# MichaelWoodhams/IQ-TREE

Hardware: AMD Instinct MI355X
Metric: million pattern-node partial-likelihood updates/sec (higher is better)
Workload: dtype f64; 1 GPU; DNA 50 taxa x 100000 patterns/GPU, GTR+G4, fixed tree: clearAllPartialLH + full traversal + root-branch lnL; ntaxa=50, patterns_per_gpu=100000, patterns_total=100000, nstates=4, ncat=4, parallelism=patterns sharded over 1 GPU(s), 1 RCCL all-reduce/step

## Files before the change

### include/iqhip.h

```cpp
#ifndef IQHIP_H_
#define IQHIP_H_

#include <stddef.h>
#include <stdint.h>

#ifdef __cplusplus
extern "C" {
#endif

#define IQHIP_ABI_VERSION 2

enum {
    IQHIP_OK = 0,
    IQHIP_ERR_NO_DEVICE = 1,
    IQHIP_ERR_INVALID = 2,
    IQHIP_ERR_UNSUPPORTED = 3,
    IQHIP_ERR_HIP = 4,
    IQHIP_ERR_NOMEM = 5
};

typedef struct iqhip_engine iqhip_engine;

typedef struct iqhip_node_op {
    uint64_t dst_key;
// ... 190 lines not shown
int iqhip_debug_pair_timing(iqhip_engine *e, double *counts_ms, double *solve_ms);

typedef struct iqhip_quartet_result {
    double  logl[3];
    double  len[3][5];
    int32_t nsweeps[3], neval[3], status[3], _pad;
} iqhip_quartet_result;
int iqhip_quartet_cells(iqhip_engine *e, const int32_t *quartets , int nq,
                        double *cells , int32_t *nother );
int iqhip_quartet_likelihoods(iqhip_engine *e, const int32_t *quartets, int nq,
                              const double *const_invar ,
                              double x1, double x2, double xacc, int max_steps, double diverge_frac,
                              int iterations, double tolerance, iqhip_quartet_result *results);
int iqhip_debug_quartet_timing(iqhip_engine *e, double *cells_ms, double *solve_ms);

typedef struct iqhip_bionj_step { int32_t a, b; double la, lb, lambda; } iqhip_bionj_step;
int iqhip_bionj(iqhip_engine *e, int n, const double *dist , const double *var ,
                iqhip_bionj_step *steps , int32_t *last , double *last_len );
int iqhip_debug_bionj_timing(iqhip_engine *e, double *ms, int64_t *launches);

typedef struct iqhip_pars_op { int32_t dst, left, right, _pad; } iqhip_pars_op;
int iqhip_pars_init(iqhip_engine *e, const uint8_t *informative , int nvectors, int64_t *nsites);
int iqhip_pars_update(iqhip_engine *e, const iqhip_pars_op *ops, int nops);
int iqhip_pars_branch_scores(iqhip_engine *e, const int32_t *ends , int nbranch, int32_t *score,
                             int32_t *subst );
int iqhip_pars_insert_scores(iqhip_engine *e, const int32_t *ends, int nbranch, int32_t taxon,
                             int32_t *score , int32_t *best, int32_t *best_score);
int iqhip_pars_shape(iqhip_engine *e, int64_t *nsites, int64_t *nwords, int *nvectors);
int iqhip_pars_fetch(iqhip_engine *e, int32_t slot, uint32_t *out );
int iqhip_debug_pars_levels(int ntaxa, int nvectors, const uint8_t *valid , const iqhip_pars_op *ops,
                            int nops, int32_t *level);
int iqhip_debug_pars_timing(iqhip_engine *e, double *ms , int64_t *counts , int reset);
int iqhip_pars_insert_scores_batch(iqhip_engine *e, const int32_t *ends ,
                                   const int32_t *seg_start , int nseg,
                                   const int32_t *taxon , int32_t *score ,
                                   int32_t *best , int32_t *best_score );
int iqhip_debug_pars_batch_timing(iqhip_engine *e, double *ms , int64_t *counts ,
                                  int reset);

enum { IQHIP_PARS_SPR_NO_SCORE = 1 };
#define IQHIP_PARS_SPR_MAX_RADIUS 10
typedef struct iqhip_pars_spr_step { int32_t parent, side, target, flags; } iqhip_pars_spr_step;
typedef struct iqhip_pars_spr_job { int32_t subtree, first_step, nsteps, _pad; } iqhip_pars_spr_job;
int iqhip_pars_spr_scan(iqhip_engine *e, const iqhip_pars_spr_job *jobs, int njobs, const iqhip_pars_spr_step *steps,
                        int nsteps, int32_t *score , int32_t *best_step ,
                        int32_t *best_score , int32_t *best_job);
int iqhip_debug_pars_spr_check(int ntaxa, int nvectors, const uint8_t *valid ,
                               const iqhip_pars_spr_job *jobs, int njobs, const iqhip_pars_spr_step *steps, int nsteps,
                               int32_t *depth );
int iqhip_debug_pars_spr_timing(iqhip_engine *e, double *ms , int64_t *counts , int reset);

int iqhip_upload_partial(iqhip_engine *e, uint64_t key, const double *partial_lh,
                         const int16_t *scale_num);

int iqhip_timing_enable(iqhip_engine *e, int on);
int iqhip_timing_read(iqhip_engine *e, double *avg_ms, int64_t *launches, int reset);
int iqhip_timing_plan_bytes(iqhip_engine *e, double *stored, double *loaded);
int iqhip_timing_collective_read(iqhip_engine *e, double *avg_us, int64_t *count, int reset);

int iqhip_debug_cherry_tables(iqhip_engine *e, int64_t *tables_built, int64_t *ops_from_tables);

#define IQHIP_PATH_NEWTON_ONE_LAUNCH 0
#define IQHIP_PATH_NEWTON_CHAIN 1
#define IQHIP_PATH_SWEEP_PERSISTENT 2
#define IQHIP_PATH_SWEEP_PER_STEP 3
#define IQHIP_PATH_SWEEP_SEQUENTIAL 4
#define IQHIP_PATH_NEWTON_FALLBACK 5
#define IQHIP_PATH_NSLOTS 6
int iqhip_debug_path_counts(iqhip_engine *e, int64_t *out, int n);

int iqhip_debug_create_planner(iqhip_engine **out, int nstates , int ncat, int64_t nptn, int ntaxa,
                               int num_cus, int state_unknown, int nclass);
int iqhip_debug_plan(iqhip_engine *e, const iqhip_node_op *ops, int nops);
#define IQHIP_PLAN_SHAPE_NSLOTS 28
int iqhip_debug_plan_shape(iqhip_engine *e, int64_t *out, int n);
#define IQHIP_PLAN_LAYOUT_NSLOTS 8
int iqhip_debug_plan_layout(iqhip_engine *e, int32_t *out, int nops);

int iqhip_debug_pair_children(iqhip_engine *e, int64_t *ops_removed, int64_t *slabs_expanded, int64_t *last_plan_removed);
int iqhip_debug_pair_rows(iqhip_engine *e, int64_t *slots_in_use, int64_t *restarts, int64_t *kept_real_for_lack_of_a_row);
int iqhip_debug_planner_plain_taxa(iqhip_engine *e, const uint8_t *plain);
int iqhip_debug_plan_removed(iqhip_engine *e, int32_t *out, int nrows);

void iqhip_debug_memory(int64_t *device_bytes, int64_t *host_bytes);
void iqhip_debug_fail_alloc(int nth);

typedef struct iqhip_partition iqhip_partition;
int iqhip_partition_create(iqhip_partition **out, iqhip_engine *const *members, int nparts);
void iqhip_partition_destroy(iqhip_partition *g);
int iqhip_partition_set_rates(iqhip_partition *g, const double *rate );
int iqhip_partition_newton_branch(iqhip_partition *g, double xguess, double x1, double x2, double xacc, int max_steps,
                                  double *optx, double *d2l, int *nsteps, double *part_lnl );
int iqhip_partition_lnl_from_theta(iqhip_partition *g, double x, double *part_lnl );
int iqhip_partition_traverse_lnl(iqhip_partition *g, const iqhip_node_op *ops, int nops, iqhip_branch_end a,
                                 iqhip_branch_end b, double len, const double *scale ,
                                 double *part_lnl );
int iqhip_partition_optimize_branch_batch(iqhip_partition *g, const iqhip_branch_task *tasks, int ntasks,
                                          iqhip_branch_result *results,
                                          double *part_lnl );
int iqhip_debug_partition_timing(iqhip_partition *g, double *ms ,
                                 int64_t *launches);

int iqhip_partition_ptnlh_reserve(iqhip_partition *g, int nrows);
int iqhip_partition_optimize_branch_batch_rows(iqhip_partition *g, const iqhip_branch_task *tasks, int ntasks,
                                               iqhip_branch_result *results,
                                               double *part_lnl ,
                                               const int32_t *rows );
int iqhip_partition_ptnlh_rell(iqhip_partition *g, const int32_t *rows, int nrows, int nsamples,
                               double *out );
int iqhip_partition_ufboot_init(iqhip_partition *g, int nsamples);
int iqhip_partition_ufboot_update(iqhip_partition *g, const iqhip_ufboot_tree *trees, int ntrees, double epsilon,
                                  double logl_cutoff, int64_t *counts , double *min_orig_logl );
int iqhip_partition_ufboot_fetch(iqhip_partition *g, double *boot_logl, double *boot_orig_logl, int32_t *boot_counts,
                                 int64_t *boot_tree);
int iqhip_debug_partition_ufboot_timing(iqhip_partition *g, double *ms , int64_t *launches);

int iqhip_partition_pair_distances(iqhip_partition *g, const double *init, double x1, double x2, double xacc, int max_steps,
                                   double *dist, double *d2l, int32_t *nsteps);
int iqhip_debug_partition_pair_timing(iqhip_partition *g, double *counts_ms, double *solve_ms);

#ifdef __cplusplus
}
#endif
#endif
```

### iq-tree_amd/__init__.py

```python
import ctypes as C
import os

import numpy as np

_HERE = os.path.dirname(os.path.abspath(__file__))
LIB_DIR = os.environ.get("IQHIP_LIB_DIR") or os.path.join(_HERE, "lib")
REPO_ROOT = os.path.dirname(_HERE)

IQHIP_SYMBOLS = [
    "iqhip_last_error", "iqhip_abi_version", "iqhip_device_count", "iqhip_create", "iqhip_destroy",
    "iqhip_set_stream", "iqhip_reserve", "iqhip_release", "iqhip_rekey", "iqhip_set_alignment",
    "iqhip_set_ptn_freq", "iqhip_set_ptn_invar", "iqhip_set_ascertainment", "iqhip_set_model", "iqhip_update_partials",
    "iqhip_branch_lnl", "iqhip_traverse_lnl", "iqhip_compute_theta", "iqhip_derv",
    "iqhip_lnl_from_theta", "iqhip_newton_branch", "iqhip_optimize_branch", "iqhip_bind_result_buffer", "iqhip_result_device_ptr",
    "iqhip_result_capacity", "iqhip_traverse_lnl_async", "iqhip_derv_async", "iqhip_result_read",
    "iqhip_synchronize", "iqhip_fetch_scale_num", "iqhip_fetch_pattern_lh", "iqhip_fetch_partial",
    "iqhip_fetch_theta", "iqhip_upload_partial", "iqhip_timing_enable", "iqhip_timing_read",
    "iqhip_fetch_pattern_lh_scaled", "iqhip_set_boot_samples", "iqhip_rell", "iqhip_rell_async",
    "iqhip_set_mixture_model", "iqhip_pattern_lh_cat", "iqhip_optimize_branch_batch",
    "iqhip_em_posteriors", "iqhip_em_fetch_posteriors", "iqhip_em_site_rates", "iqhip_em_objective", "iqhip_debug_em_timing",
    "iqhip_mix_class_lh", "iqhip_mix_weights_em", "iqhip_mix_posteriors", "iqhip_debug_mix_timing",
    "iqhip_class_lnl", "iqhip_debug_class_lnl_timing",
    "iqhip_create_sharded", "iqhip_num_shards", "iqhip_shard_range", "iqhip_comm_unique_id", "iqhip_comm_init_rank",
    "iqhip_comm_size", "iqhip_update_partials_async", "iqhip_lnl_from_theta_async",
    "iqhip_newton_host_init", "iqhip_newton_host_update", "iqhip_newton_host_result",
    "iqhip_debug_create_planner", "iqhip_debug_plan", "iqhip_timing_plan_bytes", "iqhip_timing_collective_read", "iqhip_optimize_sweep", "iqhip_debug_cherry_tables",
    "iqhip_debug_path_counts", "iqhip_debug_plan_shape", "iqhip_debug_plan_layout", "iqhip_debug_pair_children", "iqhip_debug_pair_rows", "iqhip_debug_planner_plain_taxa", "iqhip_debug_plan_removed", "iqhip_debug_memory", "iqhip_debug_fail_alloc",
    "iqhip_ptnlh_reserve", "iqhip_ptnlh_put_current", "iqhip_ptnlh_fetch", "iqhip_optimize_branch_batch_rows",
    "iqhip_branch_tests", "iqhip_ptnlh_rell",
    "iqhip_ptnlh_upload", "iqhip_gen_boot_samples", "iqhip_ptnlh_diff_variance", "iqhip_tree_tests", "iqhip_multiscale_bp",
    "iqhip_pair_counts", "iqhip_pair_distances", "iqhip_debug_pair_timing",
    "iqhip_quartet_cells", "iqhip_quartet_likelihoods", "iqhip_debug_quartet_timing",
    "iqhip_pars_init", "iqhip_pars_update", "iqhip_pars_branch_scores", "iqhip_pars_insert_scores", "iqhip_pars_fetch", "iqhip_pars_shape",
    "iqhip_debug_pars_levels", "iqhip_debug_pars_timing",
    "iqhip_pars_insert_scores_batch", "iqhip_debug_pars_batch_timing",
    "iqhip_pars_spr_scan", "iqhip_debug_pars_spr_check", "iqhip_debug_pars_spr_timing",
    "iqhip_bionj", "iqhip_debug_bionj_timing",
    "iqhip_ufboot_init", "iqhip_ufboot_update", "iqhip_ufboot_fetch", "iqhip_debug_ufboot_timing",
    "iqhip_partition_create", "iqhip_partition_destroy", "iqhip_partition_set_rates", "iqhip_partition_newton_branch",
    "iqhip_partition_lnl_from_theta", "iqhip_partition_traverse_lnl", "iqhip_debug_partition_timing",
    "iqhip_partition_optimize_branch_batch",
    "iqhip_partition_ptnlh_reserve", "iqhip_partition_optimize_branch_batch_rows", "iqhip_partition_ptnlh_rell",
    "iqhip_partition_ufboot_init", "iqhip_partition_ufboot_update", "iqhip_partition_ufboot_fetch",
    "iqhip_partition_pair_distances", "iqhip_debug_partition_pair_timing",
    "iqhip_debug_partition_ufboot_timing",
]

_LAUNCH_SLOTS = ("variant", "tab", "nfull", "ngroups", "grid", "lds_bytes", "hold_off")
PLAN_SHAPE_SLOTS = (("lds_budget", "lds_doubles", "state_slots", "nhold", "chunks", "stages") +
                    tuple("stage_units_%d" % s for s in range(8)) +
                    tuple("top_" + f for f in _LAUNCH_SLOTS) + tuple("unit_" + f for f in _LAUNCH_SLOTS))
PATH_SLOTS = ("newton_one_launch", "newton_chain", "sweep_persistent", "sweep_per_step", "sweep_sequential",
              "newton_fallback")


class NodeOp(C.Structure):
    _fields_ = [("dst_key", C.c_uint64), ("left_key", C.c_uint64), ("right_key", C.c_uint64),
                ("left_leaf", C.c_int32), ("right_leaf", C.c_int32),
                ("left_len", C.c_double), ("right_len", C.c_double), ("flags", C.c_uint32), ("_pad", C.c_uint32)]


class BranchEnd(C.Structure):
    _fields_ = [("key", C.c_uint64), ("leaf", C.c_int32), ("_pad", C.c_int32)]


class ParsOp(C.Structure):
    _fields_ = [("dst", C.c_int32), ("left", C.c_int32), ("right", C.c_int32), ("_pad", C.c_int32)]


class BranchSupport(C.Structure):
    _fields_ = [("sh_alrt", C.c_double), ("lbp", C.c_double), ("abayes", C.c_double), ("alrt_stat", C.c_double)]


class TreeTest(C.Structure):
    _fields_ = [("rell_bp", C.c_double), ("kh_pvalue", C.c_double), ("sh_pvalue", C.c_double), ("wkh_pvalue", C.c_double),
                ("wsh_pvalue", C.c_double), ("elw_value", C.c_double), ("rell_confident", C.c_int32),
                ("elw_confident", C.c_int32)]


class UFBootTree(C.Structure):
    _fields_ = [("row", C.c_int32), ("_pad", C.c_int32), ("tree_id", C.c_int64), ("logl", C.c_double), ("rand", C.c_double)]


class BranchTask(C.Structure):
    _fields_ = [("ops", C.c_void_p), ("nops", C.c_int32), ("max_steps", C.c_int32), ("a", BranchEnd), ("b", BranchEnd),
                ("xguess", C.c_double), ("x1", C.c_double), ("x2", C.c_double), ("xacc", C.c_double)]


class BranchResult(C.Structure):
    _fields_ = [("optx", C.c_double), ("d2l", C.c_double), ("lnl", C.c_double), ("nsteps", C.c_int32), ("status", C.c_int32)]


TREE_TEST_DTYPE = np.dtype([("logl", np.float64), ("rell_bp", np.float64), ("kh_pvalue", np.float64),
                            ("sh_pvalue", np.float64), ("wkh_pvalue", np.float64), ("wsh_pvalue", np.float64),
                            ("elw_value", np.float64), ("rell_confident", np.bool_), ("elw_confident", np.bool_)])
AU_SCALES = (0.5, 0.6, 0.7, 0.8, 0.9, 1.0, 1.1, 1.2, 1.3, 1.4)
BIONJ_STEP_DTYPE = np.dtype([("a", np.int32), ("b", np.int32), ("la", np.float64), ("lb", np.float64), ("lambda", np.float64)])
SUPPORT_DTYPE = np.dtype([("node1", np.int32), ("node2", np.int32), ("lh", np.float64, (3,)), ("sh_alrt", np.float64),
                          ("lbp", np.float64), ("abayes", np.float64), ("alrt_stat", np.float64)])


def leaf_end(leaf):
    return BranchEnd(0, int(leaf), 0)


def key_end(key):
    return BranchEnd(int(key), -1, 0)


ALLREDUCE_HOOK = C.CFUNCTYPE(None, C.c_void_p, C.c_int, C.c_void_p)
# ... 19 lines not shown
    lib = _load("libiqhip.so")
    if getattr(lib, "_iq_typed", False):
        return lib
    dp, ip = C.POINTER(C.c_double), C.POINTER(C.c_int16)
    vp = C.c_void_p
    lib.iqhip_last_error.restype = C.c_char_p
    lib.iqhip_create.argtypes = [C.POINTER(vp), C.c_int, C.c_int, C.c_int, C.c_int64, C.c_int]
    lib.iqhip_destroy.argtypes = [vp]
    lib.iqhip_destroy.restype = None
    lib.iqhip_set_stream.argtypes = [vp, vp]
    lib.iqhip_reserve.argtypes = [vp, C.c_int]
    lib.iqhip_release.argtypes = [vp, C.c_uint64]
    lib.iqhip_rekey.argtypes = [vp, C.c_uint64, C.c_uint64]
    lib.iqhip_set_alignment.argtypes = [vp, C.POINTER(C.c_uint8), dp, dp]
    lib.iqhip_set_ptn_freq.argtypes = [vp, dp]
    lib.iqhip_set_ptn_invar.argtypes = [vp, dp]
    lib.iqhip_set_ascertainment.argtypes = [vp, C.c_int64, C.c_double]
    lib.iqhip_set_model.argtypes = [vp, dp, dp, dp, dp, dp, C.c_int, dp]
    lib.iqhip_set_mixture_model.argtypes = [vp, C.c_int, C.POINTER(C.c_int32), dp, dp, dp, dp, dp, C.c_int, dp]
    lib.iqhip_update_partials.argtypes = [vp, C.POINTER(NodeOp), C.c_int, dp]
    lib.iqhip_branch_lnl.argtypes = [vp, BranchEnd, BranchEnd, C.c_double, dp]
    lib.iqhip_traverse_lnl.argtypes = [vp, C.POINTER(NodeOp), C.c_int, BranchEnd, BranchEnd,
                                       C.c_double, dp, dp]
    lib.iqhip_compute_theta.argtypes = [vp, BranchEnd, BranchEnd]
    lib.iqhip_derv.argtypes = [vp, C.c_double, dp, dp]
    lib.iqhip_lnl_from_theta.argtypes = [vp, C.c_double, dp]
    lib.iqhip_optimize_branch.argtypes = [vp, C.POINTER(NodeOp), C.c_int, BranchEnd, BranchEnd, C.c_double,
                                          C.c_double, C.c_double, C.c_double, C.c_int, dp, dp, dp,
                                          C.POINTER(C.c_int)]
    lib.iqhip_newton_branch.argtypes = [vp, C.c_double, C.c_double, C.c_double, C.c_double, C.c_int, dp, dp,
                                        C.POINTER(C.c_int)]
    lib.iqhip_bind_result_buffer.argtypes = [vp, vp, C.c_int]
    lib.iqhip_result_device_ptr.argtypes = [vp]
    lib.iqhip_result_device_ptr.restype = vp
    lib.iqhip_result_capacity.argtypes = [vp]
    lib.iqhip_traverse_lnl_async.argtypes = [vp, C.POINTER(NodeOp), C.c_int, BranchEnd, BranchEnd,
                                             C.c_double]
    lib.iqhip_derv_async.argtypes = [vp, C.c_double]
    lib.iqhip_result_read.argtypes = [vp, dp, C.c_int]
    lib.iqhip_synchronize.argtypes = [vp]
    lib.iqhip_fetch_scale_num.argtypes = [vp, C.c_uint64, ip]
    lib.iqhip_fetch_pattern_lh.argtypes = [vp, dp]
    lib.iqhip_fetch_partial.argtypes = [vp, C.c_uint64, dp]
    lib.iqhip_fetch_theta.argtypes = [vp, dp]
    lib.iqhip_upload_partial.argtypes = [vp, C.c_uint64, dp, ip]
    lib.iqhip_fetch_pattern_lh_scaled.argtypes = [vp, BranchEnd, BranchEnd, dp]
    lib.iqhip_set_boot_samples.argtypes = [vp, C.POINTER(C.c_float), C.c_int]
    lib.iqhip_rell.argtypes = [vp, BranchEnd, BranchEnd, dp]
    lib.iqhip_rell_async.argtypes = [vp, BranchEnd, BranchEnd]
    lib.iqhip_create_sharded.argtypes = [C.POINTER(vp), C.POINTER(C.c_int), C.c_int, C.c_int, C.c_int, C.c_int, C.c_int64,
                                         C.c_int]
    lib.iqhip_num_shards.argtypes = [vp]
    lib.iqhip_shard_range.argtypes = [vp, C.c_int, C.POINTER(C.c_int64), C.POINTER(C.c_int64), C.POINTER(C.c_int)]
    lib.iqhip_comm_unique_id.argtypes = [vp]
    lib.iqhip_comm_init_rank.argtypes = [vp, C.c_int, C.c_int, vp]
    lib.iqhip_comm_size.argtypes = [vp]
    lib.iqhip_update_partials_async.argtypes = [vp, C.POINTER(NodeOp), C.c_int]
    lib.iqhip_lnl_from_theta_async.argtypes = [vp, C.c_double]
    lib.iqhip_newton_host_init.argtypes = [vp, C.c_double, C.c_double, C.c_double, C.c_double, C.c_int, dp]
    lib.iqhip_em_posteriors.argtypes = [vp, C.c_double, dp]
    lib.iqhip_em_fetch_posteriors.argtypes = [vp, dp]
    lib.iqhip_debug_em_timing.argtypes = [vp, dp]
    lib.iqhip_em_site_rates.argtypes = [vp, dp, C.POINTER(C.c_int32)]
    lib.iqhip_em_objective.argtypes = [vp, BranchEnd, BranchEnd, C.c_double, dp, C.POINTER(C.c_int64)]
    lib.iqhip_mix_class_lh.argtypes = [vp, C.c_double, dp]
    lib.iqhip_mix_weights_em.argtypes = [vp, C.c_int, C.c_double, dp, dp, C.POINTER(C.c_int), C.POINTER(C.c_int), dp]
    lib.iqhip_mix_posteriors.argtypes = [vp, dp, dp, dp]
    lib.iqhip_debug_mix_timing.argtypes = [vp, dp, C.POINTER(C.c_int64)]
    lib.iqhip_class_lnl.argtypes = [vp, BranchEnd, BranchEnd, C.c_double, dp, dp, dp, C.POINTER(C.c_int64)]
    lib.iqhip_debug_class_lnl_timing.argtypes = [vp, dp]
    lib.iqhip_newton_host_update.argtypes = [vp, C.c_double, C.c_double, dp, C.POINTER(C.c_int)]
    lib.iqhip_newton_host_result.argtypes = [vp, dp, dp, C.POINTER(C.c_int), C.POINTER(C.c_int)]
    lib.iqhip_timing_enable.argtypes = [vp, C.c_int]
    lib.iqhip_timing_read.argtypes = [vp, dp, C.POINTER(C.c_int64), C.c_int]
    lib.iqhip_debug_create_planner.argtypes = [C.POINTER(vp), C.c_int, C.c_int, C.c_int64, C.c_int, C.c_int, C.c_int, C.c_int]
    lib.iqhip_timing_plan_bytes.argtypes = [vp, dp, dp]
    lib.iqhip_timing_collective_read.argtypes = [vp, dp, C.POINTER(C.c_int64), C.c_int]
    lib.iqhip_debug_cherry_tables.argtypes = [vp, C.POINTER(C.c_int64), C.POINTER(C.c_int64)]
    lib.iqhip_debug_path_counts.argtypes = [vp, C.POINTER(C.c_int64), C.c_int]
    lib.iqhip_debug_plan.argtypes = [vp, C.POINTER(NodeOp), C.c_int]
    lib.iqhip_debug_plan_shape.argtypes = [vp, C.POINTER(C.c_int64), C.c_int]
    lib.iqhip_debug_plan_layout.argtypes = [vp, C.POINTER(C.c_int32), C.c_int]
    lib.iqhip_debug_pair_rows.argtypes = [vp, C.POINTER(C.c_int64), C.POINTER(C.c_int64), C.POINTER(C.c_int64)]
    lib.iqhip_debug_memory.argtypes = [C.POINTER(C.c_int64), C.POINTER(C.c_int64)]
    lib.iqhip_debug_memory.restype = None
    lib.iqhip_debug_fail_alloc.argtypes = [C.c_int]
    lib.iqhip_debug_fail_alloc.restype = None
    i32p = C.POINTER(C.c_int32)
    lib.iqhip_ptnlh_reserve.argtypes = [vp, C.c_int]
    lib.iqhip_ptnlh_put_current.argtypes = [vp, C.c_int, BranchEnd, BranchEnd]
    lib.iqhip_ptnlh_fetch.argtypes = [vp, C.c_int, dp]
    lib.iqhip_optimize_branch_batch_rows.argtypes = [vp, C.POINTER(BranchTask), C.c_int, dp, C.POINTER(BranchResult), i32p]
    lib.iqhip_branch_tests.argtypes = [vp, i32p, dp, C.c_int, C.c_int, C.c_int, C.POINTER(BranchSupport)]
    lib.iqhip_ptnlh_rell.argtypes = [vp, i32p, C.c_int, C.c_int, dp]
    lib.iqhip_ptnlh_upload.argtypes = [vp, C.c_int, dp]
    lib.iqhip_gen_boot_samples.argtypes = [vp, C.c_int, C.c_int64, C.c_int64, C.c_uint64, C.c_uint32]
    lib.iqhip_ptnlh_diff_variance.argtypes = [vp, i32p, C.c_int, dp]
    lib.iqhip_tree_tests.argtypes = [vp, i32p, dp, C.c_int, C.c_int, C.c_double, C.c_int, C.c_uint64, C.POINTER(TreeTest)]
    lib.iqhip_multiscale_bp.argtypes = [vp, i32p, C.c_int, dp, C.c_int, C.c_int, C.c_uint64, dp]
    lib.iqhip_pair_counts.argtypes = [vp, i32p, C.c_int, dp]
    lib.iqhip_pair_distances.argtypes = [vp, dp, C.c_double, C.c_double, C.c_double, C.c_int, dp, dp, i32p]
    lib.iqhip_debug_pair_timing.argtypes = [vp, dp, dp]
    lib.iqhip_quartet_cells.argtypes = [vp, i32p, C.c_int, dp, i32p]
    lib.iqhip_quartet_likelihoods.argtypes = [vp, i32p, C.c_int, dp, C.c_double, C.c_double, C.c_double, C.c_int, C.c_double,
                                              C.c_int, C.c_double, vp]
    lib.iqhip_debug_quartet_timing.argtypes = [vp, dp, dp]
    u8p, u32p, i64p = C.POINTER(C.c_uint8), C.POINTER(C.c_uint32), C.POINTER(C.c_int64)
    lib.iqhip_pars_init.argtypes = [vp, u8p, C.c_int, i64p]
    lib.iqhip_pars_update.argtypes = [vp, C.POINTER(ParsOp), C.c_int]
    lib.iqhip_pars_branch_scores.argtypes = [vp, i32p, C.c_int, i32p, i32p]
    lib.iqhip_pars_insert_scores.argtypes = [vp, i32p, C.c_int, C.c_int32, i32p, i32p, i32p]
    lib.iqhip_pars_fetch.argtypes = [vp, C.c_int32, u32p]
    lib.iqhip_pars_shape.argtypes = [vp, i64p, i64p, C.POINTER(C.c_int)]
    lib.iqhip_debug_pars_levels.argtypes = [C.c_int, C.c_int, u8p, C.POINTER(ParsOp), C.c_int, i32p]
    lib.iqhip_debug_pars_timing.argtypes = [vp, dp, i64p, C.c_int]
    lib.iqhip_pars_insert_scores_batch.argtypes = [vp, i32p, i32p, C.c_int, i32p, i32p, i32p, i32p]
    lib.iqhip_debug_pars_batch_timing.argtypes = [vp, dp, i64p, C.c_int]
    lib.iqhip_pars_spr_scan.argtypes = [vp, vp, C.c_int, vp, C.c_int, i32p, i32p, i32p, i32p]
    lib.iqhip_debug_pars_spr_check.argtypes = [C.c_int, C.c_int, u8p, vp, C.c_int, vp, C.c_int, i32p]
    lib.iqhip_debug_pars_spr_timing.argtypes = [vp, dp, i64p, C.c_int]
    lib.iqhip_bionj.argtypes = [vp, C.c_int, dp, dp, vp, i32p, dp]
    lib.iqhip_debug_bionj_timing.argtypes = [vp, dp, i64p]
    lib.iqhip_ufboot_init.argtypes = [vp, C.c_int]
    lib.iqhip_ufboot_update.argtypes = [vp, C.POINTER(UFBootTree), C.c_int, C.c_double, C.c_double, i64p, dp]
    lib.iqhip_ufboot_fetch.argtypes = [vp, dp, dp, i32p, i64p]
    lib.iqhip_debug_ufboot_timing.argtypes = [vp, dp, i64p]
    lib.iqhip_partition_create.argtypes = [C.POINTER(vp), C.POINTER(vp), C.c_int]
    lib.iqhip_partition_destroy.argtypes = [vp]
    lib.iqhip_partition_destroy.restype = None
    lib.iqhip_partition_set_rates.argtypes = [vp, dp]
    lib.iqhip_partition_newton_branch.argtypes = [vp, C.c_double, C.c_double, C.c_double, C.c_double, C.c_int, dp, dp,
                                                  C.POINTER(C.c_int), dp]
    lib.iqhip_partition_lnl_from_theta.argtypes = [vp, C.c_double, dp]
    lib.iqhip_partition_traverse_lnl.argtypes = [vp, C.POINTER(NodeOp), C.c_int, BranchEnd, BranchEnd, C.c_double, dp, dp]
    lib.iqhip_partition_optimize_branch_batch.argtypes = [vp, C.POINTER(BranchTask), C.c_int, C.POINTER(BranchResult), dp]
    lib.iqhip_debug_partition_timing.argtypes = [vp, dp, i64p]
    lib.iqhip_partition_ptnlh_reserve.argtypes = [vp, C.c_int]
    lib.iqhip_partition_optimize_branch_batch_rows.argtypes = [vp, C.POINTER(BranchTask), C.c_int, C.POINTER(BranchResult), dp,
                                                               i32p]
    lib.iqhip_partition_ptnlh_rell.argtypes = [vp, i32p, C.c_int, C.c_int, dp]
    lib.iqhip_partition_ufboot_init.argtypes = [vp, C.c_int]
    lib.iqhip_partition_ufboot_update.argtypes = [vp, C.POINTER(UFBootTree), C.c_int, C.c_double, C.c_double, i64p, dp]
    lib.iqhip_partition_ufboot_fetch.argtypes = [vp, dp, dp, i32p, i64p]
    lib.iqhip_partition_pair_distances.argtypes = [vp, dp, C.c_double, C.c_double, C.c_double, C.c_int, dp, dp, i32p]
    lib.iqhip_debug_partition_pair_timing.argtypes = [vp, dp, dp]
    lib.iqhip_debug_partition_ufboot_timing.argtypes = [vp, dp, i64p]
    lib._iq_typed = True
    return lib


def libiqhost():
    libiqhip()
    lib = _load("libiqhost.so")
    if getattr(lib, "_iq_typed", False):
        return lib
    dp, vp = C.POINTER(C.c_double), C.c_void_p
    lib.iqhost_last_error.restype = C.c_char_p
    lib.iqhost_create.argtypes = [C.POINTER(vp), C.c_char_p, C.POINTER(C.c_char_p), C.c_int]
    lib.iqhost_destroy.argtypes = [vp]
    lib.iqhost_destroy.restype = None
    lib.iqhost_set_alignment.argtypes = [vp, C.c_int, C.c_int, C.c_int64, C.POINTER(C.c_uint8), dp, dp]
    lib.iqhost_set_ascertainment.argtypes = [vp, C.c_int64, C.c_double]
    lib.iqhost_set_ptn_freq.argtypes = [vp, dp]
    lib.iqhost_set_ptn_invar.argtypes = [vp, dp]
    lib.iqhost_set_model.argtypes = [vp, C.c_int, dp, dp, dp, dp, dp]
    lib.iqhost_set_mixture_model.argtypes = [vp, C.c_int, C.c_int, C.POINTER(C.c_int), dp, dp, dp, dp, dp]
# ... 2529 lines not shown
```

### iq-tree_amd/csrc/engine.hip

```cpp
#include <math.h>
#include <stdio.h>
#include <stdlib.h>
#include <string.h>

#include <algorithm>
#include <cmath>
#include <atomic>

#include "iqhip_internal.h"

using namespace iqhip;

static thread_local std::string g_err;
namespace iqhip {
int set_error(int code, const std::string &msg) {
    g_err = msg;
    return code;
}
double debug_build_us = 0.0;
}

extern "C" void iqhip_debug_memory(int64_t *device_bytes, int64_t *host_bytes) {
    if (device_bytes) *device_bytes = g_mem_bytes[0].load();
    if (host_bytes) *host_bytes = g_mem_bytes[1].load();
// ... 468 lines not shown
    e->d_inv_evec = d_model + o_ievec;
    e->d_rates = d_model + o_rates;
    e->d_props = d_model + o_props;
    e->d_tip = d_model + o_tip;
    e->d_evalc = d_model + o_evalc;
    e->d_tipc = d_model + o_tipc;
    e->d_cls = reinterpret_cast<int *>(d_model + o_cls);
    e->d_aimg = aimg_doubles ? d_model + o_aimg : nullptr;
    e->aimg_doubles = (int)aimg_doubles;
    if (nclass > 1 || (e->n == 20 && !e->mfma_pipelined_ok) || e->wide4) {
        const int MT = (n + 15) / 16, KS = n / 4;
        const size_t mix_doubles = (size_t)nclass * 4 * KS * 64;
        std::vector<double> img(mix_doubles + (size_t)nclass * 2 * MT * KS * 64, 0.0);
        for (int m = 0; m < nclass; m++) {
            const double *U = evec + (size_t)m * n * n, *Ui = inv_evec + (size_t)m * n * n;
            for (int s = 0; s < KS; s++)
                for (int l = 0; l < 64; l++) {
                    const int k = 4 * s + (l >> 4), r16 = l & 15, r4 = 16 + (l & 3);
                    double *b = &img[(size_t)m * 4 * KS * 64];
                    if (r16 < n) {
                        b[(0 * KS + s) * 64 + l] = U[r16 * n + k];
                        b[(2 * KS + s) * 64 + l] = Ui[r16 * n + k];
                    }
                    if (r4 < n) {
                        b[(1 * KS + s) * 64 + l] = U[r4 * n + k];
                        b[(3 * KS + s) * 64 + l] = Ui[r4 * n + k];
                    }
                }
            for (int t = 0; t < MT * KS * 64; t++) {
                const int l = t & 63, ms = t >> 6, s = ms % KS, mt = ms / KS;
                const int row = 16 * mt + (l & 15), k = 4 * s + (l >> 4);
                if (row < n) {
                    img[mix_doubles + ((size_t)m * 2 + 0) * MT * KS * 64 + t] = U[row * n + k];
                    img[mix_doubles + ((size_t)m * 2 + 1) * MT * KS * 64 + t] = Ui[row * n + k];
                }
            }
        }
        e->img_generic_off = mix_doubles;
        HIPCHK(e->d_img.ensure(e, img.size()));
        HIPCHK(hipMemcpy(e->d_img.p, img.data(), sizeof(double) * img.size(), hipMemcpyHostToDevice));
    }
    const bool pipelined = e->mfma_pipelined_ok && nclass == 1;
    if (pipelined != e->mfma_pipelined || nclass != e->nclass) {
        e->mfma_pipelined = pipelined;
        e->plan_cache.invalidate();
    }
    e->h_props.assign(props, props + e->ncat);
    e->h_cls = cls;
    e->nclass = nclass;
    e->state_unknown = state_unknown;
    e->model_set = true;
    e->theta_valid = false;
    e->model_version++;
    e->cherry_model_synced = false;
    return IQHIP_OK;
}

bool iqhip::cherry_candidate(const iqhip_engine *e) {
    if (!e || !e->cherry_on || !e->shards.empty()) return false;
    if (!e->mfma_pipelined_ok || e->n_user != e->n) return false;
    if (e->n == 20) return e->ncat == 4 && !e->leaf_tables && !e->cat_split && e->nptn_pad >= 8 * 1024;
    return false;
}

static int cherry_sync_model(iqhip_engine *e, const double *eval, const double *evec, const double *inv_evec,
                             const double *rates, const double *props, int state_unknown, const double *tip) {
    const int s2 = state_unknown + 1;
    if (s2 * s2 > 4356 || (int64_t)4 * s2 * s2 > e->nptn_pad) {
        if (e->pair) iqhip_destroy(e->pair);
        e->pair = nullptr;
        return IQHIP_OK;
    }
    if (e->pair && e->cherry_s2 != s2) {
        HIPCHK(hipStreamSynchronize(e->stream));
        iqhip_destroy(e->pair);
        e->pair = nullptr;
    }
    int rc = IQHIP_OK;
    if (!e->pair) {
        const int npairs = s2 * s2;
        rc = iqhip_create(&e->pair, e->device, e->n, e->ncat, npairs, 2);
        if (rc) return rc;
        e->pair->cherry_on = false;
        e->pair->check_plans = e->check_plans;
        rc = iqhip_set_stream(e->pair, e->stream);
        if (rc) return rc;
        e->cherry_s2 = s2;
        e->cherry_npairs = (int)e->pair->nptn_pad;
        e->cherry_slot_of.clear();
        e->cherry_slots.clear();
    }
    rc = set_model_common(e->pair, 1, nullptr, eval, evec, inv_evec, rates, props, state_unknown, tip);
    if (rc) return rc;
    if (!e->pair->aln_set) {
        const int npairs = s2 * s2;
        std::vector<uint8_t> st((size_t)2 * npairs);
        for (int q = 0; q < npairs; q++) {
            st[q] = (uint8_t)(q / s2);
            st[(size_t)npairs + q] = (uint8_t)(q % s2);
        }
        const std::vector<double> ones((size_t)npairs, 1.0), zeros((size_t)npairs, 0.0);
        rc = iqhip_set_alignment(e->pair, st.data(), ones.data(), zeros.data());
    }
    return rc;
}

static int set_model_binary(iqhip_engine *e, const double *eval, const double *evec, const double *inv_evec,
                            const double *rates, const double *props, int state_unknown, const double *tip) {
    if (!eval || !evec || !inv_evec || !rates || !props || !tip) return fail(IQHIP_ERR_INVALID, "null argument");
    const int m = e->n_user, n = e->n;
    if (state_unknown != m)
        return fail(IQHIP_ERR_INVALID, "iqhip_set_model: data of this state count has STATE_UNKNOWN = nstates (no ambiguity codes)");
    std::vector<double> ev((size_t)n, 0.0), U((size_t)n * n, 0.0), Ui((size_t)n * n, 0.0), tp((size_t)(n + 2) * n, 0.0);
    for (int i = 0; i < m; i++) ev[i] = eval[i];
    for (int x = 0; x < m; x++)
        for (int i = 0; i < m; i++) { U[(size_t)x * n + i] = evec[x * m + i]; Ui[(size_t)x * n + i] = inv_evec[x * m + i]; }
    for (int x = m; x < n; x++) U[(size_t)x * n + x] = Ui[(size_t)x * n + x] = 1.0;
    for (int st = 0; st < m; st++)
        for (int i = 0; i < m; i++) tp[(size_t)st * n + i] = tip[st * m + i];
    for (int i = 0; i < m; i++) tp[(size_t)n * n + i] = tp[(size_t)(n + 1) * n + i] = tip[m * m + i];
    return set_model_common(e, 1, nullptr, ev.data(), U.data(), Ui.data(), rates, props, n + 1, tp.data());
}

extern "C" int iqhip_set_model(iqhip_engine *e, const double *eval, const double *evec,
                               const double *inv_evec, const double *rates, const double *props,
                               int state_unknown, const double *tip_partial_lh) {
    if (e && e->embed2 && e->shards.empty())
        return set_model_binary(e, eval, evec, inv_evec, rates, props, state_unknown, tip_partial_lh);
    int rc = set_model_common(e, 1, nullptr, eval, evec, inv_evec, rates, props, state_unknown, tip_partial_lh);
    if (!rc) e->mixture_api = false;
    if (!rc && cherry_candidate(e)) {
        rc = cherry_sync_model(e, eval, evec, inv_evec, rates, props, state_unknown, tip_partial_lh);
        e->cherry_model_synced = !rc && e->pair != nullptr;
    }
    return rc;
}

extern "C" int iqhip_set_mixture_model(iqhip_engine *e, int nclass, const int32_t *cat_class, const double *eval,
                                       const double *evec, const double *inv_evec, const double *rates,
                                       const double *props, int state_unknown, const double *tip_partial_lh) {
    if (e && (e->embed2 || (e->n_user != 4 && e->n_user != 20 && e->n_user != 64)) && nclass > 1)
        return fail(IQHIP_ERR_UNSUPPORTED, "mixture models of embedded data (state counts other than 4, 20, 64) are not implemented");
    if (e && e->embed2 && e->shards.empty())
        return set_model_binary(e, eval, evec, inv_evec, rates, props, state_unknown, tip_partial_lh);
    const int rc = set_model_common(e, nclass, cat_class, eval, evec, inv_evec, rates, props, state_unknown, tip_partial_lh);
    if (!rc) e->mixture_api = true;
    return rc;
}

int iqhip::ensure_slab_rows(iqhip_engine *e, int nrows) {
    HIPCHK(e->d_slab.ensure(e, (size_t)nrows * e->ntiles * e->lane_split));
    return IQHIP_OK;
}

int iqhip::check_ready(iqhip_engine *e) {
    if (!e) return fail(IQHIP_ERR_INVALID, "null engine");
    if (!e->model_set || !e->aln_set)
        return fail(IQHIP_ERR_INVALID, "engine needs iqhip_set_model and iqhip_set_alignment first");
    hipError_t s = use_device(e);
    if (s != hipSuccess) return fail(IQHIP_ERR_HIP, hipGetErrorString(s));
    return IQHIP_OK;
}

int iqhip::require(iqhip_engine *e, const char *what, unsigned needs) {
    const auto no = [what](int code, const char *why) { return fail(code, std::string(what) + ": " + why); };
    if (!e) return no(IQHIP_ERR_INVALID, "null engine");
// ... 26 lines not shown
    }
    hipEventRecord(e->tev[e->tev_used].first, e->stream);
}
static void timing_end(iqhip_engine *e) {
    if (!e->timing) return;
    hipEventRecord(e->tev[e->tev_used].second, e->stream);
    e->tev_used++;
}

static int build_cherry_tables(iqhip_engine *e) {
    iqhip_engine *p = e->pair;
    const int n = (int)e->plan.cherry_jobs.size();
    std::vector<iqhip_node_op> ops((size_t)n);
    const std::vector<int> segs((size_t)n, 1);
    for (int i = 0; i < n; i++) {
        const iqhip_engine::CherrySlot &cs = e->cherry_slots[e->plan.cherry_jobs[i]];
        iqhip_node_op &o = ops[i];
        memset(&o, 0, sizeof o);
        o.dst_key = (uint64_t)e->plan.cherry_jobs[i] + 1;
        o.left_leaf = 0;
        o.right_leaf = 1;
        o.left_len = cs.len_l;
        o.right_len = cs.len_r;
    }
    iqhip_branch_end none = {0, -1, 0};
    int rc = submit_traverse(p, ops.data(), n, false, none, none, 0.0, true, &segs, nullptr);
    if (rc) return rc;
    std::vector<const double *> src((size_t)n);
    std::vector<double *> dst((size_t)n);
    const size_t per = (size_t)e->cherry_npairs * e->block;
    for (int i = 0; i < n; i++) {
        int idx;
        rc = slab_for_key(p, ops[i].dst_key, false, &idx);
        if (rc) return rc;
        src[i] = p->slabs[idx].plh.p;
        dst[i] = e->d_cherry_tab.p + (size_t)e->plan.cherry_jobs[i] * per;
    }
    HIPCHK(launch_cherry_transpose(e, src.data(), dst.data(), n, e->cherry_npairs));
    for (int i = 0; i < n; i++) e->cherry_slots[e->plan.cherry_jobs[i]].model_version = e->model_version;
    e->cherry_built_total += n;
    e->plan.cherry_jobs.clear();
    return IQHIP_OK;
}

int iqhip::submit_traverse(iqhip_engine *e, const iqhip_node_op *ops, int nops, bool has_root,
                           iqhip_branch_end a, iqhip_branch_end b, double len, bool skip_reduce,
                           const std::vector<int> *explicit_segs, const double *const *len_ptrs) {
    int rc = check_ready(e);
    if (rc) return rc;
    if (nops < 0 || (nops > 0 && !ops)) return fail(IQHIP_ERR_INVALID, "bad ops array");
    int last_dst = -1;
    Stopwatch watch;
    if (e->debug_sweep) watch.start();
    e->n_root_end_keys = 0;
    if (has_root) {
        if (a.leaf < 0) e->root_end_keys[e->n_root_end_keys++] = a.key;
        if (b.leaf < 0) e->root_end_keys[e->n_root_end_keys++] = b.key;
    }
    rc = build_plan(e, ops, nops, &last_dst, explicit_segs, len_ptrs);
    e->n_root_end_keys = 0;
    if (rc) return rc;
    if (e->debug_sweep) debug_build_us += watch.us();
    DevBranch br;
    if (has_root) {
        rc = build_branch(e, a, b, len, last_dst, &br);
        if (rc) return rc;
    }
    rc = ensure_slab_rows(e, 2 + nops);
    if (rc) return rc;
    const int nwaves = (int)e->ntiles * e->lane_split;
    if (e->plan.nleaf_tabs > 0) {
        const int njobs = leaf_tables_follow_model(e) ? e->plan.nleaf_tabs : e->plan.tab_dirty;
        if (njobs > 0)
            HIPCHK(launch_leaf_tables(e, reinterpret_cast<const TabJob *>(e->d_ops.p + e->plan.jobs_off), njobs));
        e->plan.tab_dirty = 0;
    }
    if (!e->plan.cherry_jobs.empty()) {
        rc = build_cherry_tables(e);
        if (rc) return rc;
    }
    if (e->plan.uses_cherry)
        for (int k = 0; k < nops; k++) e->cherry_ops_total += e->h_ops.p[k].cherry != nullptr;
    timing_begin(e);
    const int *table = reinterpret_cast<const int *>(e->d_ops.p + e->plan.table_off);
    {
        int off = 2;
        for (int n : e->plan.stage_units) {
            if (e->mfma) HIPCHK(launch_traverse_mfma(e, table + off, n, nwaves));
            else HIPCHK(launch_traverse4(e, table + off, n, e->plan.units_have_load, nullptr, nwaves));
            off += 2 * n;
        }
    }
    const bool empty_top = e->plan.nunits > 0 && !has_root && e->plan.top_nops == 0;
    const bool fold4 = e->fold_reduce && !e->mfma && !empty_top && !skip_reduce;
    const bool foldm = e->fold_reduce && e->mfma && has_root && e->n_unobs == 0;
    if (empty_top) {
    } else if (e->mfma) HIPCHK(launch_traverse_mfma(e, table, nops > 0 ? 1 : 0, nwaves, true));
    else HIPCHK(launch_traverse4(e, table, 1, e->plan.has_load, has_root ? &br : nullptr, nwaves, fold4 ? nops : -1));
    timing_end(e);
    if (e->timing) e->tev_launches += (int)e->plan.stage_units.size() + (empty_top ? 0 : 1);
    if (e->mfma && has_root) HIPCHK(launch_stream_mfma(e, 0, &br, br.len, nwaves, nullptr, foldm ? nops : -1));
    if (fold4 || foldm) {
    } else if (has_root) HIPCHK(launch_reduce(e, 0, 2 + nops, nwaves));
    else if (!skip_reduce) HIPCHK(launch_reduce(e, 2, nops, nwaves));
    e->last_nops = nops;
    e->last_has_root = has_root;
    e->last_root_loads_b = has_root && br.b_kind != CHILD_PREV;
    return IQHIP_OK;
}

int iqhip::read_result(iqhip_engine *e, int ndoubles) {
    if (e->d_result != e->d_result_own)
        HIPCHK(hipMemcpyAsync(e->h_result.p, e->d_result, sizeof(double) * ndoubles, hipMemcpyDeviceToHost,
                              e->stream));
    else if (e->poll_pending) {
        e->poll_pending = false;
        const unsigned long long want = e->result_seq;
        for (int spin = 0; spin < 200000; spin++) {
            if (*e->h_done.p == want) {
                std::atomic_thread_fence(std::memory_order_acquire);
                e->staging_busy = false;
                if (e->folded_rows >= 0) {
                    if (e->h_result.p[2 + e->folded_rows] == 0.0)
                        for (int k = 0; k < e->folded_rows; k++) e->h_result.p[2 + k] = 0.0;
                    e->folded_rows = -1;
                }
                return IQHIP_OK;
            }
            __builtin_ia32_pause();
        }
    }
    e->poll_pending = false;
    HIPCHK(hipStreamSynchronize(e->stream));
    e->staging_busy = false;
    if (e->folded_rows >= 0) {
        if (e->h_result.p[2 + e->folded_rows] == 0.0)
            for (int k = 0; k < e->folded_rows; k++) e->h_result.p[2 + k] = 0.0;
        e->folded_rows = -1;
    }
    return IQHIP_OK;
}

void iqhip::result_arrived(iqhip_engine *e) {
    e->poll_pending = false;
    e->staging_busy = false;
    if (e->folded_rows >= 0) {
        if (e->h_result.p[2 + e->folded_rows] == 0.0)
            for (int k = 0; k < e->folded_rows; k++) e->h_result.p[2 + k] = 0.0;
        e->folded_rows = -1;
    }
}

static int repair_lnl(iqhip_engine *e, double *lnl) {
    std::vector<double> plh((size_t)e->nptn_pad), freq((size_t)e->nptn_pad);
    HIPCHK(hipMemcpy(plh.data(), e->d_pattern_lh.p, sizeof(double) * plh.size(), hipMemcpyDeviceToHost));
    HIPCHK(hipMemcpy(freq.data(), e->d_freq.p, sizeof(double) * freq.size(), hipMemcpyDeviceToHost));
    double s = 0.0;
    for (int64_t p = 0; p < e->nptn; p++) {
        if (isnan(plh[p]) || isinf(plh[p])) plh[p] = kLogScalingThreshold * 4;
        s += plh[p] * freq[p];
    }
    HIPCHK(hipMemcpy(e->d_pattern_lh.p, plh.data(), sizeof(double) * plh.size(), hipMemcpyHostToDevice));
    *lnl = s;
    return IQHIP_OK;
}

// ... 90 lines not shown
    e->theta_valid = true;
    e->theta_a_sc = br.a_sc;
    e->theta_b_sc = br.b_sc;
    if (b.leaf >= 0) std::swap(a, b);
    e->theta_end[0] = a;
    e->theta_end[1] = b;
}

extern "C" int iqhip_compute_theta(iqhip_engine *e, iqhip_branch_end a, iqhip_branch_end b) {
    if (e && !e->shards.empty()) return sharded::compute_theta(e, a, b);
    int rc = check_ready(e);
    if (rc) return rc;
    DevBranch br;
    rc = build_branch(e, a, b, 0.0, -1, &br);
    if (rc) return rc;
    if (e->mfma) HIPCHK(launch_stream_mfma(e, 1, &br, 0.0, (int)e->ntiles));
    else HIPCHK(launch_theta4(e, br));
    set_theta_branch(e, br, a, b);
    return IQHIP_OK;
}

extern "C" int iqhip_derv_async(iqhip_engine *e, double len) {
    if (e && !e->shards.empty())
        return fail(IQHIP_ERR_UNSUPPORTED, "a sharded engine reduces its results itself: use the synchronous calls");
    int rc = check_ready(e);
    if (rc) return rc;
    if (!e->theta_valid) return fail(IQHIP_ERR_INVALID, "iqhip_derv: theta not computed");
    if (!(len >= 0.0)) return fail(IQHIP_ERR_INVALID, "negative or NaN branch length");
    const int nrows = e->n_unobs > 0 ? 5 : 2;
    if (e->asc_active && e->n_unobs == 0) {
        if (e->d_result == e->d_result_own) e->h_result.p[2] = e->h_result.p[3] = e->h_result.p[4] = 0.0;
        else HIPCHK(hipMemsetAsync(e->d_result + 2, 0, 3 * sizeof(double), e->stream));
    }
    rc = ensure_slab_rows(e, nrows);
    if (rc) return rc;
    const int nwaves = (int)e->ntiles;
    if (e->mfma) HIPCHK(launch_stream_mfma(e, 2, nullptr, len, nwaves));
    else HIPCHK(launch_derv4(e, len, nwaves));
    HIPCHK(launch_reduce(e, 0, nrows, nwaves));
    return IQHIP_OK;
}

extern "C" int iqhip_derv(iqhip_engine *e, double len, double *df, double *ddf) {
    if (e && !e->shards.empty()) return sharded::derv(e, len, df, ddf);
    int rc = iqhip_derv_async(e, len);
    if (rc) return rc;
    rc = comm_allreduce(e, e->asc_active ? 5 : 2);
    if (rc) return rc;
    rc = read_result(e, e->asc_active ? 5 : 2);
    if (rc) return rc;
    double a = e->h_result.p[0], b = e->h_result.p[1];
    newton_repair(a, b);
    if (e->asc_active) asc_derv_correct(e->h_result.p + 2, e->asc_nsites, a, b);
    if (df) *df = a;
    if (ddf) *ddf = b;
    return IQHIP_OK;
}

extern "C" int iqhip_debug_cherry_tables(iqhip_engine *e, int64_t *tables_built, int64_t *ops_from_tables) {
    if (!e) return fail(IQHIP_ERR_INVALID, "null engine");
    if (tables_built) *tables_built = e->cherry_built_total;
    if (ops_from_tables) *ops_from_tables = e->cherry_ops_total;
    return IQHIP_OK;
}

extern "C" int iqhip_debug_pair_children(iqhip_engine *e, int64_t *ops_removed, int64_t *slabs_expanded, int64_t *last_plan_removed) {
    if (!e) return fail(IQHIP_ERR_INVALID, "null engine");
    if (!e->shards.empty()) e = e->shards[0];
    if (ops_removed) *ops_removed = e->pair_ops_removed;
    if (slabs_expanded) *slabs_expanded = e->pair_slabs_expanded;
    if (last_plan_removed) *last_plan_removed = (int64_t)e->plan.virt.size();
    return IQHIP_OK;
}

extern "C" int iqhip_debug_pair_rows(iqhip_engine *e, int64_t *slots_in_use, int64_t *restarts, int64_t *kept_real_for_lack_of_a_row) {
    if (!e) return fail(IQHIP_ERR_INVALID, "null engine");
    if (!e->shards.empty()) e = e->shards[0];
    if (slots_in_use) *slots_in_use = (int64_t)e->pair_row_of.size();
    if (restarts) *restarts = e->pair_row_restarts;
    if (kept_real_for_lack_of_a_row) *kept_real_for_lack_of_a_row = e->pair_ops_without_row;
    return IQHIP_OK;
}

extern "C" int iqhip_debug_planner_plain_taxa(iqhip_engine *e, const uint8_t *plain) {
    if (!e || !e->planner) return fail(IQHIP_ERR_INVALID, "iqhip_debug_planner_plain_taxa needs a planning-only engine");
    e->taxon_plain.clear();
    if (plain) e->taxon_plain.assign(plain, plain + e->ntaxa);
    e->plan_cache.invalidate();
    return IQHIP_OK;
}

extern "C" int iqhip_debug_plan_removed(iqhip_engine *e, int32_t *out, int nrows) {
    if (!e || !e->planner || !out || nrows != e->plan.nrows)
        return fail(IQHIP_ERR_INVALID, "iqhip_debug_plan_removed needs a planning-only engine and the last plan's row count");
    std::fill(out, out + nrows, 1);
    for (int k = 0; k < e->plan.small_nops; k++) out[e->h_ops.p[k].out_row] = 0;
    return IQHIP_OK;
}

extern "C" int iqhip_debug_path_counts(iqhip_engine *e, int64_t *out, int n) {
    if (!e) return fail(IQHIP_ERR_INVALID, "null engine");
    if (!out && n > 0) return fail(IQHIP_ERR_INVALID, "null argument");
    for (int k = 0; k < n && k < IQHIP_PATH_NSLOTS; k++) out[k] = e->path_counts[k];
    return IQHIP_OK;
}

extern "C" int iqhip_lnl_from_theta_async(iqhip_engine *e, double len) {
    if (e && !e->shards.empty())
        return fail(IQHIP_ERR_UNSUPPORTED, "a sharded engine reduces its results itself: use the synchronous calls");
    int rc = check_ready(e);
    if (rc) return rc;
    if (!e->theta_valid) return fail(IQHIP_ERR_INVALID, "iqhip_lnl_from_theta: theta not computed");
    if (!(len >= 0.0)) return fail(IQHIP_ERR_INVALID, "negative or NaN branch length");
    rc = ensure_slab_rows(e, 2);
    if (rc) return rc;
    const int nwaves = (int)e->ntiles;
    if (e->mfma) HIPCHK(launch_stream_mfma(e, 3, nullptr, len, nwaves));
    else HIPCHK(launch_lnl_theta4(e, len, nwaves));
    HIPCHK(launch_reduce(e, 0, 2, nwaves));
    return IQHIP_OK;
}

extern "C" int iqhip_lnl_from_theta(iqhip_engine *e, double len, double *lnl) {
    if (e && !e->shards.empty()) return sharded::lnl_from_theta(e, len, lnl);
    int rc = iqhip_lnl_from_theta_async(e, len);
    if (rc) return rc;
    rc = comm_allreduce(e, e->asc_active ? 2 : 1);
    if (rc) return rc;
    rc = read_result(e, 2);
    if (rc) return rc;
    double v = e->h_result.p[0];
    if (isnan(v) || isinf(v)) {
        rc = repair_lnl_comm(e, &v);
        if (rc) return rc;
    }
    rc = asc_finish_lnl(e, &v);
    if (rc) return rc;
    if (lnl) *lnl = v;
    return IQHIP_OK;
}

extern "C" int iqhip_bind_result_buffer(iqhip_engine *e, void *device_ptr, int capacity_doubles) {
    if (!e) return fail(IQHIP_ERR_INVALID, "null engine");
    if (!e->shards.empty() || e->comm)
        return fail(IQHIP_ERR_UNSUPPORTED, "an engine with a communicator reduces in its own device result vector");
    HIPCHK(use_device(e));
    HIPCHK(hipStreamSynchronize(e->stream));
    if (!device_ptr) {
        e->d_result = e->d_result_own;
        e->result_cap = 8 + 16384;
        return IQHIP_OK;
    }
    if (capacity_doubles < 2) return fail(IQHIP_ERR_INVALID, "result buffer too small");
    e->d_result = (double *)device_ptr;
    e->result_cap = std::min(capacity_doubles, 8 + 16384);
    return IQHIP_OK;
}
extern "C" void *iqhip_result_device_ptr(iqhip_engine *e) { return (e && e->shards.empty()) ? (void *)e->d_result : nullptr; }
extern "C" int iqhip_result_capacity(iqhip_engine *e) { return e ? e->result_cap : 0; }

extern "C" int iqhip_result_read(iqhip_engine *e, double *out, int ndoubles) {
    if (e && !e->shards.empty())
        return fail(IQHIP_ERR_UNSUPPORTED, "a sharded engine reduces its results itself: use the synchronous calls");
    if (!e || !out || ndoubles < 0 || ndoubles > e->result_cap)
        return fail(IQHIP_ERR_INVALID, "iqhip_result_read: bad arguments");
    HIPCHK(use_device(e));
// ... 167 lines not shown
    }
    if (stored) *stored = st;
    if (loaded) *loaded = ld;
    return IQHIP_OK;
}

extern "C" int iqhip_timing_read(iqhip_engine *e, double *avg_ms, int64_t *launches, int reset) {
    if (!e) return fail(IQHIP_ERR_INVALID, "null engine");
    if (!e->shards.empty()) {
        double worst = 0.0;
        int64_t n0 = 0;
        for (size_t g = 0; g < e->shards.size(); g++) {
            double a = 0.0;
            int64_t n = 0;
            int rc = iqhip_timing_read(e->shards[g], &a, &n, reset);
            if (rc) return rc;
            if (a > worst) worst = a;
            if (g == 0) n0 = n;
        }
        if (avg_ms) *avg_ms = worst;
        if (launches) *launches = n0;
        return IQHIP_OK;
    }
    HIPCHK(use_device(e));
    HIPCHK(hipStreamSynchronize(e->stream));
    double total = 0.0;
    for (size_t i = 0; i < e->tev_used; i++) {
        float ms = 0.f;
        HIPCHK(hipEventElapsedTime(&ms, e->tev[i].first, e->tev[i].second));
        total += ms;
    }
    if (avg_ms) *avg_ms = e->tev_launches ? total / (double)e->tev_launches : 0.0;
    if (launches) *launches = e->tev_launches;
    if (reset) { e->tev_used = 0; e->tev_launches = 0; }
    return IQHIP_OK;
}

extern "C" int iqhip_debug_create_planner(iqhip_engine **out, int nstates, int ncat, int64_t nptn, int ntaxa, int num_cus,
                                          int state_unknown, int nclass) {
    if (!out) return fail(IQHIP_ERR_INVALID, "iqhip_debug_create_planner: out == NULL");
    *out = nullptr;
    if (nptn <= 0 || ntaxa < 2 || ncat < 1 || num_cus < 1 || nclass < 1 || nclass > ncat)
        return fail(IQHIP_ERR_INVALID, "iqhip_debug_create_planner: bad shape");
    if (nstates != 4 && nstates != 20 && nstates != 64)
        return fail(IQHIP_ERR_UNSUPPORTED, "iqhip_debug_create_planner: nstates must be 4, 20 or 64");
    if (state_unknown < nstates || state_unknown > 255) return fail(IQHIP_ERR_INVALID, "state_unknown out of range");
    {
        const int rc = check_shape4("iqhip_debug_create_planner", nstates, nstates, ncat);
        if (rc) return rc;
    }
    iqhip_engine *e = new iqhip_engine();
    e->planner = true;
    e->check_plans = true;
    e->num_cus = num_cus;
    configure_engine(e, -1, nstates, nstates, ncat, nptn, ntaxa);
    const size_t P = (size_t)e->nptn_pad;
    e->d_states.ensure(e, (size_t)ntaxa * P);
    e->dummy.plh.ensure(e, P * e->block);
    e->dummy.sc.ensure(e, P);
    e->result_cap = 8 + 16384;
    e->state_unknown = state_unknown;
    e->nclass = nclass;
    if (nclass > 1 && nstates == 4 && !e->wide4) {
        e->mfma = true;
        e->lane_split = 1;
        e->tile = 16;
        e->ntiles = e->nptn_pad / 16;
    }
    e->mfma_pipelined = e->mfma_pipelined_ok && nclass == 1;
    e->model_set = e->aln_set = true;
    {
        const int s2 = state_unknown + 1;
        if (cherry_candidate(e) && nclass == 1 && s2 * s2 <= 4356 && (int64_t)4 * s2 * s2 <= e->nptn_pad) {
            e->cherry_s2 = s2;
            e->cherry_npairs = (int)round_up(s2 * s2, 64);
        }
    }
    *out = e;
    return IQHIP_OK;
}

extern "C" int iqhip_debug_plan(iqhip_engine *e, const iqhip_node_op *ops, int nops) {
    if (!e || !e->planner) return fail(IQHIP_ERR_INVALID, "iqhip_debug_plan needs a planning-only engine");
    if (nops < 0 || (nops > 0 && !ops)) return fail(IQHIP_ERR_INVALID, "bad ops array");
    int last_dst = -1;
    const int rc = build_plan(e, ops, nops, &last_dst, nullptr);
    if (!rc) {
        e->cherry_built_total += (int64_t)e->plan.cherry_jobs.size();
        for (int slot : e->plan.cherry_jobs) e->cherry_slots[slot].model_version = e->model_version;
        e->plan.cherry_jobs.clear();
        for (int k = 0; k < nops; k++) e->cherry_ops_total += e->h_ops.p[k].cherry != nullptr;
    }
    return rc;
}

extern "C" int iqhip_debug_plan_shape(iqhip_engine *e, int64_t *out, int n) {
    if (!e || !e->planner || !out || n < IQHIP_PLAN_SHAPE_NSLOTS)
        return fail(IQHIP_ERR_INVALID, "iqhip_debug_plan_shape needs a planning-only engine and IQHIP_PLAN_SHAPE_NSLOTS slots");
    std::fill(out, out + n, (int64_t)0);
    const Plan &p = e->plan;
    const int nops = p.small_nops;
    int chunks = 0;
    for (int k = 0; k < nops; k += e->h_ops.p[k].chunk_nops) chunks++;
    out[0] = lds_budget(e); out[1] = p.lds_doubles; out[2] = p.state_slots; out[3] = p.nhold; out[4] = chunks;
    out[5] = (int64_t)p.stage_units.size();
    for (size_t s = 0; s < p.stage_units.size() && s < 8; s++) out[6 + s] = p.stage_units[s];
    auto launch = [&](int64_t *o, bool top_stage, int nsegs) {
        TravLaunch L = {TRAV_NONE, false, 0, 0, 0, 0, -1};
        if (e->mfma) L = choose_traverse_mfma(e, top_stage, nsegs);
        else {
            L.variant = (TravVariant)-1;
            L.ngroups = trav4_ngroups(e);
            L.grid = L.ngroups * nsegs;
            L.lds_bytes = trav4_lds_bytes(e->block, p.lds_doubles, p.state_slots);
        }
        const int64_t v[7] = {L.variant, L.tab, L.nfull, L.ngroups, L.grid, (int64_t)L.lds_bytes, L.hold_off};
        std::copy(v, v + 7, o);
    };
    launch(out + 14, true, nops > 0 ? 1 : 0);
    if (!p.stage_units.empty()) launch(out + 21, false, p.stage_units[0]);
    return IQHIP_OK;
}

extern "C" int iqhip_debug_plan_layout(iqhip_engine *e, int32_t *out, int nops) {
    if (!e || !e->planner || !out || nops != e->plan.small_nops)
        return fail(IQHIP_ERR_INVALID, "iqhip_debug_plan_layout needs a planning-only engine and the last plan's op count");
    for (int k = 0; k < nops; k++) {
        const DevOp &d = e->h_ops.p[k];
        const int32_t v[IQHIP_PLAN_LAYOUT_NSLOTS] = {d.chunk_nops, d.chunk_slots, d.left_kind == CHILD_LEAF, d.right_kind == CHILD_LEAF,
                                                     d.lds_left, d.lds_right, d.sl_slot, d.sr_slot};
        std::copy(v, v + IQHIP_PLAN_LAYOUT_NSLOTS, out + (size_t)k * IQHIP_PLAN_LAYOUT_NSLOTS);
    }
    return IQHIP_OK;
}
```

### iq-tree_amd/csrc/iqhip_internal.h

```cpp
#pragma once
#include <hip/hip_runtime.h>
#include <stdint.h>
#include <stdlib.h>
#include <time.h>
#include <algorithm>
#include <atomic>
#include <string>
#include <type_traits>
#include <unordered_map>
#include <vector>
#include "../../include/iqhip.h"
#include "trav_lds.h"

namespace iqhip {

constexpr int kSmallPlanOps = 4;
constexpr int kNewtonPostEpochs = 128;
constexpr int kMixEmTile = 256;
constexpr int kMixEmRegClasses = 8;
constexpr int kMixEmBatch = 16;
constexpr int kMixEmUpdateThreads = 1024;
constexpr double kScalingThreshold = 0x1p-256;
constexpr double kScalingThresholdInv = 0x1p256;
constexpr double kLogScalingThreshold = -177.44567822334599;

enum ChildKind : int32_t { CHILD_LEAF = 0, CHILD_LOAD = 1, CHILD_PREV = 2, CHILD_PF = 3, CHILD_HOLD = 4, CHILD_PAIR = 5 };
constexpr bool child_is_table(int32_t kind) { return kind == CHILD_LEAF || kind == CHILD_PAIR; }
constexpr int kPairRows = 25;
constexpr int child_region_blocks(int32_t kind) { return kind == CHILD_LEAF ? 6 : (kind == CHILD_PAIR ? 1 + kPairRows + 12 : 1); }

struct __attribute__((aligned(16))) DevOp {
    double *dst;
    int16_t *dst_sc;
    const double *pf;
    const int16_t *pf_sc;
    const uint8_t *sl;
    const uint8_t *sr;
    const double *ld;
    const int16_t *ld_sc;
    int32_t left_kind;
    int32_t right_kind;
    double left_len;
    double right_len;
    int32_t lds_left;
    int32_t lds_right;
    int32_t chunk_nops;
    int32_t real_mask;
    int32_t sl_slot;
    int32_t sr_slot;
    int32_t push_hold;
    int32_t out_row;
    int32_t no_scale;
    const double *tabL;
    const double *tabR;
    const double *left_len_p;
    const double *right_len_p;
    const double *cherry;
    int32_t chunk_slots;
    int32_t _pad_slots;
    double pair_len[4];
    int32_t pair_row_l, pair_row_r;
};

#if defined(__HIPCC__)
__device__ __forceinline__ double wave_sum64(double v) {
    unsigned lo = __double2loint(v), hi = __double2hiint(v);
    auto a = __builtin_amdgcn_permlane32_swap(lo, lo, false, false);
    auto b = __builtin_amdgcn_permlane32_swap(hi, hi, false, false);
    v = __hiloint2double(b[0], a[0]) + __hiloint2double(b[1], a[1]);
    lo = __double2loint(v);
    hi = __double2hiint(v);
    auto c = __builtin_amdgcn_permlane16_swap(lo, lo, false, false);
    auto d = __builtin_amdgcn_permlane16_swap(hi, hi, false, false);
    v = __hiloint2double(d[0], c[0]) + __hiloint2double(d[1], c[1]);
#define IQHIP_DPP_STEP(ctrl)                                                                                  \
    v += __hiloint2double(__builtin_amdgcn_mov_dpp(__double2hiint(v), ctrl, 0xF, 0xF, true),                  \
                          __builtin_amdgcn_mov_dpp(__double2loint(v), ctrl, 0xF, 0xF, true));
    IQHIP_DPP_STEP(0x128)
    IQHIP_DPP_STEP(0x124)
    IQHIP_DPP_STEP(0x4E)
    IQHIP_DPP_STEP(0xB1)
#undef IQHIP_DPP_STEP
    return v;
}

__device__ __forceinline__ double group_sum(double v) {
    unsigned lo = __double2loint(v), hi = __double2hiint(v);
    auto a = __builtin_amdgcn_permlane16_swap(lo, lo, false, false);
    auto b = __builtin_amdgcn_permlane16_swap(hi, hi, false, false);
    v = __hiloint2double(b[0], a[0]) + __hiloint2double(b[1], a[1]);
    lo = __double2loint(v);
    hi = __double2hiint(v);
    auto c = __builtin_amdgcn_permlane32_swap(lo, lo, false, false);
    auto d = __builtin_amdgcn_permlane32_swap(hi, hi, false, false);
    return __hiloint2double(d[0], c[0]) + __hiloint2double(d[1], c[1]);
}

constexpr unsigned kScalingThresholdHi = 0x2FF00000u;
__device__ __forceinline__ unsigned amax_hi(unsigned m, double v) {
    const unsigned h = (unsigned)__double2hiint(v) & 0x7fffffffu;
    return m > h ? m : h;
}
__device__ __forceinline__ unsigned nonzero_bits(double v) {
    return ((unsigned)__double2hiint(v) & 0x7fffffffu) | (unsigned)__double2loint(v);
}
__device__ __forceinline__ unsigned group_max_u(unsigned v) {
    auto a = __builtin_amdgcn_permlane32_swap(v, v, false, false);
    v = a[0] > a[1] ? a[0] : a[1];
    auto b = __builtin_amdgcn_permlane16_swap(v, v, false, false);
    return b[0] > b[1] ? b[0] : b[1];
}

template <typename OpRef>
__device__ __forceinline__ double op_child_len(const OpRef &d, int child) {
    const double *p = child ? d.right_len_p : d.left_len_p;
    return p ? *p : (child ? d.right_len : d.left_len);
}
#endif

struct __attribute__((aligned(16))) DevBranch {
    const double *a;
    const uint8_t *a_states;
    const double *b;
    const int16_t *a_sc;
    const int16_t *b_sc;
    int32_t a_kind;
    int32_t b_kind;
    double len;
};

struct __attribute__((aligned(16))) SweepOp {
    double *dst;
    int16_t *dst_sc;
    const double *lv, *rv;
    const int16_t *lsc, *rsc;
    const uint8_t *ls, *rs;
    double llen, rlen;
    int32_t llen_step, rlen_step;
    int32_t no_scale;
    int32_t row;
};
struct __attribute__((aligned(16))) SweepStep {
    DevBranch br;
    double xguess;
    int32_t op_begin, nops;
};

struct __attribute__((aligned(16))) PairTile {
    int32_t ra[4], rb[4];
    int32_t out[16];
};

struct __attribute__((aligned(16))) TabJob {
    double len;
    double *tab;
    const double *len_p;
    double _pad;
};

struct Plan {
    int lds_doubles = 0;
    int state_slots = 1;
    bool has_load = false;
    bool units_have_load = false;
    bool small = false;
    int small_nops = 0;
    int nunits = 0, top_nops = 0;
    std::vector<int> stage_units;
    int table_off = 0, jobs_off = 0;
    int nhold = 0;
    int nleaf_tabs = 0;
    std::vector<TabJob> tab_jobs;
    int tab_dirty = 0;
    std::vector<int> cherry_jobs;
    bool uses_cherry = false;
    uint64_t cherry_model = 0;
    struct Virtual { int slab; int32_t taxon_l, taxon_r; double len_l, len_r; };
    std::vector<Virtual> virt;
    int nrows = 0;
};

struct PlanCache {
    std::vector<char> ops_in;
    std::vector<int> segs;
    uint64_t version = 0;
    int dst = -1;
    std::vector<char> uploaded;
    void invalidate() { version = 0; uploaded.clear(); }
};

struct __attribute__((aligned(16))) NewtonState {
    double x1, x2, xacc;
    double rts, rts_old, xl, xh, dx, f, df, d2l, result;
    int32_t max_steps, j, neval, status;
    int32_t done, _pad[3];
};

__host__ __device__ inline void newton_init(NewtonState &s, double xguess, double x1, double x2, double xacc,
                                            int max_steps) {
    s.x1 = x1; s.x2 = x2; s.xacc = xacc;
    s.rts = xguess;
    if (s.rts < x1) s.rts = x1;
    if (s.rts > x2) s.rts = x2;
    s.rts_old = s.rts; s.xl = x1; s.xh = x2; s.dx = 0.0; s.f = s.df = s.d2l = 0.0;
    s.result = s.rts;
    s.max_steps = max_steps; s.j = 0; s.neval = 0; s.status = 0; s.done = 0;
    s._pad[0] = s._pad[1] = s._pad[2] = 0;
}

__host__ __device__ inline bool newton_finite(double v) { return v == v && v - v == 0.0; }

__host__ __device__ inline void newton_repair(double &pdf, double &pddf) {
    if (!newton_finite(pdf)) { pdf = 0.0; pddf = 0.0; }
}

__host__ __device__ inline void asc_derv_correct(const double *c, double asc_nsites, double &df, double &ddf) {
    const double prob_const = 1.0 - c[0];
    const double df_frac = c[1] / prob_const, ddf_frac = c[2] / prob_const;
    df += asc_nsites * df_frac;
    ddf += asc_nsites * (ddf_frac + df_frac * df_frac);
}

__host__ __device__ inline void newton_advance(NewtonState &s, double f, double df) {
    if (s.done) return;
    s.f = f; s.df = df;
    s.neval++;
    if (s.neval == 1) {
        s.d2l = df;
        if (!newton_finite(f) || !newton_finite(df)) { s.status = 2; s.result = s.rts; s.done = 1; return; }
        if (df >= 0.0 && fabs(f) < s.xacc) { s.result = s.rts; s.done = 1; return; }
        if (f < 0.0) { s.xl = s.rts; s.xh = s.x2; } else { s.xh = s.rts; s.xl = s.x1; }
        s.dx = fabs(s.xh - s.xl);
        s.j = 1;
    } else {
        if (!newton_finite(f) || !newton_finite(df)) { s.status = 2; s.result = s.rts_old; s.done = 1; return; }
        if (df > 0.0 && fabs(f) < s.xacc) { s.d2l = df; s.result = s.rts; s.done = 1; return; }
        if (f < 0.0) s.xl = s.rts; else s.xh = s.rts;
        s.j++;
        if (s.j > s.max_steps) { s.status = 3; s.result = s.rts; s.done = 1; return; }
    }
    s.rts_old = s.rts;
    if ((df <= 0.0) || (((s.rts - s.xh) * df - f) * ((s.rts - s.xl) * df - f) >= 0.0)) {
        s.dx = 0.5 * (s.xh - s.xl);
        s.rts = s.xl + s.dx;
        s.d2l = df;
        if (s.xl == s.rts) { s.result = s.rts; s.done = 1; return; }
    } else {
        s.dx = f / df;
        const double temp = s.rts;
        s.rts -= s.dx;
        s.d2l = df;
        if (temp == s.rts) { s.result = s.rts; s.done = 1; return; }
    }
    if (fabs(s.dx) < s.xacc || s.j == s.max_steps) { s.result = s.rts_old; s.done = 1; return; }
}

__host__ __device__ inline void newton_update(NewtonState &s, double pdf, double pddf) {
    if (s.done) return;
    newton_repair(pdf, pddf);
    newton_advance(s, -pdf, -pddf);
}

// ... 226 lines not shown
        iqhip::DevBuf<iqhip::PairTile> tiles;
        iqhip::DevBuf<double> counts, coef, init, out;
        double ms[2] = {0.0, 0.0};
    } pd;
    struct {
        iqhip::DevBuf<int32_t> quartets, nother, other;
        iqhip::DevBuf<double> cells;
        iqhip::DevBuf<iqhip_quartet_result> out;
        double ms[2] = {0.0, 0.0};
    } qt;
    struct {
        double ms = 0.0;
        int64_t launches = 0;
    } bj;
    std::vector<double> h_freq, h_evec0, h_tip0;
    bool pars_ready = false;
    int pars_nvec = 0;
    int64_t pars_nsites = 0, pars_nwords = 0;
    std::vector<uint8_t> pars_valid;
    struct {
        iqhip::DevBuf<uint32_t> vec, score;
        iqhip::DevBuf<int32_t> ints;
        iqhip::DevBuf<int32_t> out;
        iqhip::DevBuf<uint64_t> masks;
    } pars;
    iqhip::PinBuf<int32_t> h_pars_ops, h_pars_ends, h_pars_out;
    double pars_ms[2] = {0.0, 0.0};
    int64_t pars_counts[4] = {0, 0, 0, 0};
    double pars_spr_ms = 0.0;
    int64_t pars_spr_counts[2] = {0, 0};
    double pars_batch_ms = 0.0;
    int64_t pars_batch_counts[3] = {0, 0, 0};
    iqhip::DevBuf<int32_t> d_batch_rows;
    double *d_result_own = nullptr, *d_result = nullptr;
    iqhip::DevBuf<double> d_newton_partials;
    iqhip::DevBuf<unsigned int> d_newton_barrier;
    unsigned int newton_launches = 0;
    iqhip::DevBuf<double> d_newton_posts;
    unsigned int newton_post_launches = 0;
    bool newton_posts = true;
    iqhip::DevBuf<double> d_batch_posts;
    size_t batch_posts_used[2] = {0, 0};
    unsigned int batch_post_launches = 0;
    iqhip::DevBuf<double> d_theta_batch, d_batch_partials, d_batch_out;
    iqhip::DevBuf<unsigned int> d_batch_barriers;
    iqhip::DevBuf<char> d_batch_tasks;
    int batch_cap = 0;
    unsigned int batch_launches = 0;
    iqhip::DevBuf<double> d_sweep_len;
    iqhip::PinBuf<char> h_sweep_desc;
    iqhip::DevBuf<char> d_sweep_desc;
    iqhip::DevBuf<unsigned long long> d_sweep_prof;
    iqhip::DevBuf<double> d_sweep_posts;
    int num_cus = 256;
    int result_cap = 0;
    void *comm = nullptr;
    int comm_nranks = 1, comm_rank = 0;
    iqhip::DevBuf<double> d_result_dev;
    iqhip::DevBuf<iqhip::NewtonState> d_nstate;
    iqhip::PinBuf<iqhip::NewtonState> h_nstate;
    iqhip::DevBuf<iqhip::NewtonState> d_bstates;
    iqhip::DevBuf<const int16_t *> d_bsc;
    std::vector<iqhip_engine *> shards;
    std::vector<int64_t> shard_first;
    int reduce_mode = 0;
    iqhip::PinBuf<iqhip::DevOp> h_ops;
    iqhip::PinBuf<double> h_result;
    iqhip::PlanCache plan_cache;
    iqhip::PinBuf<char> h_plan_arena;
    size_t plan_arena_used = 0;
    bool plan_arena_on = false;
    uint64_t keymap_version = 1;
    hipEvent_t staging_free = nullptr;
    bool staging_busy = false;

    std::vector<char> taxon_plain;
    uint64_t root_end_keys[2] = {0, 0};
    int n_root_end_keys = 0;
    iqhip::DevBuf<uint8_t> d_pair_rows;
    std::unordered_map<uint64_t, int> pair_row_of;
    int64_t pair_ops_removed = 0, pair_slabs_expanded = 0;
    int64_t pair_row_restarts = 0, pair_ops_without_row = 0;

    std::unordered_map<uint64_t, int> key2slab;
    std::vector<iqhip::Slab> slabs;
    std::vector<int> free_slabs;

    bool timing = false;
    std::vector<std::pair<hipEvent_t, hipEvent_t>> tev;
    size_t tev_used = 0;
    std::vector<std::pair<hipEvent_t, hipEvent_t>> cev;
    size_t cev_used = 0;
    int64_t tev_launches = 0;
    int last_nops = 0;
    bool last_has_root = false, last_root_loads_b = false;
    int folded_rows = -1;
};

namespace iqhip {

struct FoldArgs {
    double *slab;
    double *result;
    unsigned int *ticket;
    int *flags;
    int nwaves;
    int nrows_scale;
    int root_rows;
    int enabled;
    volatile unsigned long long *done;
    unsigned long long seq;
};

#if defined(__HIPCC__)
__device__ __forceinline__ void fold_store(double *p, double v) {
    __hip_atomic_store(p, v, __ATOMIC_RELAXED, __HIP_MEMORY_SCOPE_AGENT);
}
__device__ __forceinline__ void fold_flag(const FoldArgs &F, int row) {
    __hip_atomic_fetch_or(&F.flags[row], 1, __ATOMIC_RELAXED, __HIP_MEMORY_SCOPE_AGENT);
}

__device__ inline void fold_tail(const FoldArgs &F) {
    __shared__ double s_f[256];
    __shared__ int s_last;
    asm volatile("s_waitcnt vmcnt(0)" ::: "memory");
    __syncthreads();
    if (threadIdx.x == 0) {
        const unsigned int t = __hip_atomic_fetch_add(F.ticket, 1u, __ATOMIC_RELAXED, __HIP_MEMORY_SCOPE_AGENT);
        s_last = (t == gridDim.x - 1) ? 1 : 0;
    }
    __syncthreads();
    if (!s_last) return;
    __shared__ int s_rows[256];
    __shared__ int s_n;
    const int nrows = 2 + F.nrows_scale;
    auto sum_row = [&](int row) {
        const double *r = F.slab + (size_t)row * F.nwaves;
        if (threadIdx.x < 64) {
            double acc[4] = {0.0, 0.0, 0.0, 0.0};
            for (int base = 0; base < F.nwaves; base += 8 * 256) {
                double v[4][8];
#pragma unroll
                for (int j = 0; j < 4; j++)
#pragma unroll
                    for (int q = 0; q < 8; q++) {
                        const int i = base + q * 256 + (int)threadIdx.x + 64 * j;
                        v[j][q] = i < F.nwaves ? __hip_atomic_load(&r[i], __ATOMIC_RELAXED, __HIP_MEMORY_SCOPE_AGENT) : 0.0;
                    }
#pragma unroll
                for (int j = 0; j < 4; j++)
#pragma unroll
                    for (int q = 0; q < 8; q++) {
                        const int i = base + q * 256 + (int)threadIdx.x + 64 * j;
                        if (i < F.nwaves) acc[j] += v[j][q];
                    }
            }
#pragma unroll
            for (int j = 0; j < 4; j++) s_f[(int)threadIdx.x + 64 * j] = acc[j];
        }
        __syncthreads();
#pragma unroll
        for (int o = 128; o > 0; o >>= 1) {
            if (threadIdx.x < 64)
                for (int v = (int)threadIdx.x; v < o; v += 64) s_f[v] += s_f[v + o];
            __syncthreads();
        }
// ... 41 lines not shown
    }
    if (F.done && threadIdx.x == 0) F.result[nrows] = (double)nflagged;
    if (threadIdx.x == 0) {
        __hip_atomic_store(F.ticket, 0u, __ATOMIC_RELAXED, __HIP_MEMORY_SCOPE_AGENT);
        if (F.done) {
            __threadfence_system();
            *F.done = F.seq;
        }
    }
}
#endif

int set_error(int code, const std::string &msg);
inline int fail(int code, const std::string &msg) { return set_error(code, msg); }
#define HIPCHK(call)                                                                                           \
    do {                                                                                                       \
        hipError_t _s = (call);                                                                                \
        if (_s != hipSuccess)                                                                                  \
            return iqhip::set_error(IQHIP_ERR_HIP, std::string(#call) + ": " + hipGetErrorString(_s));        \
    } while (0)

template <typename T>
T *fake_alloc(iqhip_engine *e, size_t count) {
    const uint64_t a = e->fake_next;
    e->fake_next += (count * sizeof(T) + 255) / 256 * 256 + 256;
    return reinterpret_cast<T *>(a);
}
template <typename T>
hipError_t DevBuf<T>::ensure(iqhip_engine *e, size_t count) {
    if (!e->planner) return ensure(e->stream, count);
    if (count > this->cap) {
        this->p = fake_alloc<T>(e, count);
        this->cap = count;
    }
    return hipSuccess;
}
template <typename T>
hipError_t PinBuf<T>::ensure(iqhip_engine *e, size_t count, bool mapped) {
    if (!e->planner) return ensure(e->stream, count, mapped);
    return count <= this->cap ? hipSuccess : this->replace(nullptr, count, MEM_HOST);
}
constexpr unsigned kLdsCeilingDevices = 64;
template <auto Kernel>
hipError_t raise_lds_ceiling(const iqhip_engine *e, int bytes) {
    static std::atomic<bool> raised[kLdsCeilingDevices];
    const unsigned dev = (unsigned)e->device;
    if (dev < kLdsCeilingDevices && raised[dev].load(std::memory_order_relaxed)) return hipSuccess;
    const hipError_t s = hipFuncSetAttribute(reinterpret_cast<const void *>(Kernel), hipFuncAttributeMaxDynamicSharedMemorySize, bytes);
    if (s == hipSuccess && dev < kLdsCeilingDevices) raised[dev].store(true, std::memory_order_relaxed);
    return s;
}
struct PhaseTimer {
    PhaseTimer(iqhip_engine *e_, int nphases_) : e(e_), nphases(nphases_), ok(e_->timing) {}
    PhaseTimer(const PhaseTimer &) = delete; PhaseTimer &operator=(const PhaseTimer &) = delete;
    void mark() {
        hipEvent_t x = nullptr;
        if (!ok || !(ok = hipEventCreate(&x) == hipSuccess)) return;
        ev.push_back(x);
        ok = hipEventRecord(x, e->stream) == hipSuccess;
    }
    bool read(double *ms) {
        const size_t round = (size_t)nphases + 1;
        if (!ok || ev.empty() || ev.size() % round || hipEventSynchronize(ev.back()) != hipSuccess) return false;
        std::vector<double> sum((size_t)nphases, 0.0);
        for (size_t k = 0; k < ev.size(); k += round)
            for (int h = 0; h < nphases; h++) {
                float t = 0.0f;
                if (hipEventElapsedTime(&t, ev[k + h], ev[k + h + 1]) != hipSuccess) return false;
                sum[(size_t)h] += t;
            }
        std::copy(sum.begin(), sum.end(), ms);
        return true;
    }
    ~PhaseTimer() { for (hipEvent_t x : ev) hipEventDestroy(x); }
    iqhip_engine *e;
    int nphases;
    bool ok;
    std::vector<hipEvent_t> ev;
};
int slab_for_key(iqhip_engine *e, uint64_t key, bool create, int *idx);
int expand_virtual_slabs(iqhip_engine *e);
hipError_t launch_pair_expand(iqhip_engine *e, const Slab &s);
hipError_t launch_pair_codes(iqhip_engine *e, const uint8_t *row_l, const uint8_t *row_r, uint8_t *out);
bool cherry_candidate(const iqhip_engine *e);

int build_plan(iqhip_engine *e, const iqhip_node_op *ops, int nops, int *last_dst,
               const std::vector<int> *explicit_segs = nullptr, const double *const *len_ptrs = nullptr);
int build_branch(iqhip_engine *e, iqhip_branch_end a, iqhip_branch_end b, double len, int prev_dst, DevBranch *br);
int resolve_child(iqhip_engine *e, uint64_t key, int32_t leaf, int prev_dst, const double **plh, const int16_t **sc,
                  const uint8_t **states, int32_t *kind);
bool leaf_tables_follow_model(iqhip_engine *e);
int lds_budget(const iqhip_engine *e);

enum TravVariant : int {
    TRAV_NONE = 0,
    TRAV_GENERIC,
    TRAV_MIX20,
    TRAV_MIX20_SPLIT,
    TRAV_M2,
    TRAV_M2_CAT_SPLIT,
    TRAV_M2_TOP_CS2,
    TRAV_TOP20,
    TRAV_ROWS64,
    TRAV_TOP64,
    TRAV_WIDE4,
};
struct TravLaunch {
    TravVariant variant;
    bool tab;
    int nfull;
    int ngroups;
    int grid;
    size_t lds_bytes;
    int hold_off;
};
TravLaunch choose_traverse_mfma(const iqhip_engine *e, bool top_stage, int nsegs);
inline bool top_stage_may_share_tiles(const iqhip_engine *e) { return e->top_cs2; }
inline bool top_stage_may_mix_roles64(const iqhip_engine *e) { return e->n == 64 && e->mixed_top; }
inline int trav4_ngroups(const iqhip_engine *e) {
    const int wpb = kTravWg / 64;
    return (int)((e->ntiles * e->lane_split + wpb - 1) / wpb);
}
inline bool kernel_takes_small_plan(const iqhip_engine *e) {
    return !e->mfma || (e->mfma_pipelined && e->n == 20 && !e->leaf_tables && e->plan.nleaf_tabs == 0);
}

int comm_allreduce(iqhip_engine *e, int n);
int comm_group_allreduce(const std::vector<iqhip_engine *> &shards, int n);
int comm_init_all(const std::vector<iqhip_engine *> &shards);
void comm_destroy(iqhip_engine *e);
int comm_use_device_result(iqhip_engine *e);

hipError_t use_device(const iqhip_engine *e);
enum : unsigned {
    REQ_SINGLE_DEVICE = 1u << 0,
    REQ_NO_ASC = 1u << 1,
    REQ_PLAIN_STATES = 1u << 2,
    REQ_STATES_4_20_64 = 1u << 3,
    REQ_STATES_4 = 1u << 4,
    REQ_NO_MIXTURE = 1u << 5,
    REQ_MIXTURE = 1u << 6,
    REQ_MODEL_ALN = 1u << 7,
    REQ_THETA = 1u << 8,
};
int require(iqhip_engine *e, const char *what, unsigned needs);
int check_ready(iqhip_engine *e);
int branch_scale_counters(iqhip_engine *e, iqhip_branch_end a, iqhip_branch_end b, const int16_t *sc[2]);
int ensure_slab_rows(iqhip_engine *e, int nrows);
int submit_traverse(iqhip_engine *e, const iqhip_node_op *ops, int nops, bool has_root, iqhip_branch_end a,
                    iqhip_branch_end b, double len, bool skip_reduce = false, const std::vector<int> *explicit_segs = nullptr,
                    const double *const *len_ptrs = nullptr);
int read_result(iqhip_engine *e, int ndoubles);
void set_theta_branch(iqhip_engine *e, const DevBranch &br, iqhip_branch_end a, iqhip_branch_end b);
void result_arrived(iqhip_engine *e);
int eng_repair_lnl(iqhip_engine *e, double *lnl);
extern double debug_build_us;

struct Stopwatch {
    timespec t0;
    void start() { clock_gettime(CLOCK_MONOTONIC, &t0); }
    double us() const {
        timespec t1;
        clock_gettime(CLOCK_MONOTONIC, &t1);
        return (t1.tv_sec - t0.tv_sec) * 1e6 + (t1.tv_nsec - t0.tv_nsec) * 1e-3;
    }
};
// ... 310 lines not shown
```

### iq-tree_amd/csrc/kernels_valu4.hip

```cpp
#include "iqhip_internal.h"
#include "trav_phases.h"

namespace iqhip {

#define CONST_AS __attribute__((address_space(4)))
template <typename T>
__device__ __forceinline__ const CONST_AS T *as_const(const T *p) {
    return (const CONST_AS T *)(p);
}

__device__ __forceinline__ double wave_sum(double v) { return wave_sum64(v); }

template <int C>
__device__ __forceinline__ void load_vec4(const double *__restrict__ base, int64_t tile, int lane,
                                          double (&v)[4 * C]) {
    const double2 *p = reinterpret_cast<const double2 *>(base + tile * (64 * 4 * C)) + lane;
#pragma unroll
    for (int j = 0; j < 2 * C; j++) {
        double2 t = p[j * 64];
        v[2 * j] = t.x;
        v[2 * j + 1] = t.y;
    }
}
template <int C>
__device__ __forceinline__ void store_vec4(double *__restrict__ base, int64_t tile, int lane,
                                           const double (&v)[4 * C]) {
    double2 *p = reinterpret_cast<double2 *>(base + tile * (64 * 4 * C)) + lane;
#pragma unroll
    for (int j = 0; j < 2 * C; j++) p[j * 64] = make_double2(v[2 * j], v[2 * j + 1]);
}

struct Trav4Args {
    const DevOp *ops;
    const double *evec;
    const double *inv_evec;
    const double *tip;
    const double *freq;
    const double *invar;
    const double *eval;
    const double *rates;
    const double *props;
    double *pattern_lh;
    double *slab;
    int64_t ntiles;
    int64_t nptn;
    int64_t nobs;
    const int *segs;
    int ngroups;
    int nwaves;
    int state_unknown;
    int has_root;
    int lds_reg_doubles;
    int state_slots;
    int nsegs_launch;
    int has_load;
    FoldArgs fold;
    DevBranch root;
    int small_plan;
    int small_segs[2];
    DevOp small_ops[kSmallPlanOps];
};

template <int CF>
__device__ __forceinline__ void leaf_cat4(const double *reg , const double *s_tip,
                                          const CONST_AS double *U, int s, int row, bool slow,
                                          int state_unknown, int c, double (&a)[4]) {
    constexpr int B = 4 * CF;
    if (__builtin_expect(slow, 0)) {
        double l[4];
#pragma unroll
        for (int i = 0; i < 4; i++) l[i] = reg[c * 4 + i] * s_tip[s * 4 + i];
#pragma unroll
        for (int x = 0; x < 4; x++) {
            double v = U[x * 4] * l[0];
            v = fma(U[x * 4 + 1], l[1], v);
            v = fma(U[x * 4 + 2], l[2], v);
            v = fma(U[x * 4 + 3], l[3], v);
            a[x] = (s == state_unknown) ? 1.0 : v;
        }
    } else {
        const double2 *tab = reinterpret_cast<const double2 *>(reg + B + row * B + c * 4);
        const double2 v0 = tab[0], v1 = tab[1];
        a[0] = v0.x; a[1] = v0.y; a[2] = v1.x; a[3] = v1.y;
    }
}

template <int C, int CF>
__device__ __forceinline__ double node_update4(bool leafL, bool holdL, bool leafR, bool pairL, bool pairR, const double *regL,
                                               const double *regR, const double *s_tip,
                                               const CONST_AS double *U, const CONST_AS double *uinv,
                                               int sL, int sR, int state_unknown, const char *nx_pf,
                                               char *dst, int coff, double (&PF)[4 * C],
                                               const double (&HOLD)[4 * C], double (&prev)[4 * C]) {
    bool slowL = false, slowR = false;
    int rowL = 0, rowR = 0;
    if (leafL) {
        slowL = !pairL && __any((sL >= 4) && (sL != state_unknown));
        rowL = pairL ? sL : (sL < 4 ? sL : 4);
    }
    if (leafR) {
        slowR = !pairR && __any((sR >= 4) && (sR != state_unknown));
        rowR = pairR ? sR : (sR < 4 ? sR : 4);
    }
    double lh_max = 0.0;
#pragma unroll
    for (int c = 0; c < C; c++) {
        double a[4], b[4], tmp[4];
        if (leafL) {
            leaf_cat4<CF>(regL, s_tip, U, sL, rowL, slowL, state_unknown, coff + c, a);
        } else {
            double l[4];
            if (holdL) {
#pragma unroll
                for (int i = 0; i < 4; i++) l[i] = regL[(coff + c) * 4 + i] * HOLD[c * 4 + i];
            } else {
#pragma unroll
                for (int i = 0; i < 4; i++) l[i] = regL[(coff + c) * 4 + i] * PF[c * 4 + i];
            }
#pragma unroll
            for (int x = 0; x < 4; x++) {
                double v = U[x * 4] * l[0];
                v = fma(U[x * 4 + 1], l[1], v);
                v = fma(U[x * 4 + 2], l[2], v);
                a[x] = fma(U[x * 4 + 3], l[3], v);
// ... 108 lines not shown
    const uint32_t voff = (uint32_t)(tl * (64 * B * 8) + pl * 16 + coff * 2048);
    const uint32_t doff = (uint32_t)(lane * 16);
    const uint32_t soff = (uint32_t)(ptn * 2);
    const uint32_t poff = (uint32_t)ptn;

    const double freq = A.freq[ptn];
    const double invar = A.invar[ptn];

    const CONST_AS double *U = as_const(A.evec);
    const CONST_AS double *uinv = as_const(A.inv_evec);
    const CONST_AS DevOp *ops = A.small_plan ? (const CONST_AS DevOp *)(kargs + offsetof(Trav4Args, small_ops)) : as_const(A.ops);

    double prev[BL], PF[BL], HOLD[BL];
    int hold_sc = 0;
    int pf_sc = 0, prev_sc = 0;
#pragma unroll
    for (int e = 0; e < BL; e++) { prev[e] = 0.0; PF[e] = 0.0; }
#pragma unroll
    for (int e = 0; e < BL; e++) HOLD[e] = 0.0;

    if (active) {
        const CONST_AS DevOp *nx = ops + k_begin;
        const int nreal = nx->real_mask;
        load_vec4_off<CL>(nx->pf, (nreal & 1) ? voff : doff, PF);
        pf_sc = *reinterpret_cast<const int16_t *>(reinterpret_cast<const char *>(nx->pf_sc) +
                                                   ((nreal & 1) ? soff : (uint32_t)(lane * 2)));
    }


#ifdef IQHIP_T4_TRACE
    const bool t4_on = (blockIdx.x % 97) == 5 && threadIdx.x == 0;
    unsigned long long t4_fill = 0, t4_head = 0, t4_upd = 0, t4_tail = 0, t4_n = 0, t4_f1 = 0, t4_f2 = 0;
#endif
    int k = k_begin;
    while (k < k_end) {
        const int kn = ops[k].chunk_nops;
        const int nslots = ops[k].chunk_slots;
        [[maybe_unused]] const unsigned long long c0 = T4_CLK();
        __syncthreads();
        if (threadIdx.x == 0) s_npair = 0;
        for (int t = threadIdx.x; t < kn; t += kTravWg) {
            const CONST_AS DevOp &d = ops[k + t];
            const int slot_l = d.sl_slot, slot_r = d.sr_slot;
            const uint8_t *const row_l = d.sl, *const row_r = d.sr;
            s_row[slot_l] = row_l;
            s_row[slot_r] = row_r;
        }
        auto request_states = [&]() {
            if constexpr (SP == 1) {
                if (active) {
                    constexpr int RB = 4;
                    const int grp = lane >> 4;
                    const int64_t roff = tl * 64 + 4 * (lane & 15);
                    for (int s0 = 1; s0 < nslots; s0 += 4 * RB) {
                        const uint8_t *row[RB];
#pragma unroll
                        for (int r = 0; r < RB; r++) {
                            const int slot = s0 + 4 * r + grp;
                            row[r] = s_row[slot < nslots ? slot : 0];
                        }
#pragma unroll
                        for (int r = 0; r < RB; r++) {
                            if (s0 + 4 * r + grp < nslots)
                                __builtin_amdgcn_global_load_lds((const __attribute__((address_space(1))) void *)(row[r] + roff),
                                                                 (__attribute__((address_space(3))) void *)(w_states + (s0 + 4 * r) * 64), 4, 0, 0);
                        }
                    }
                }
            }
        };
        lds_barrier();
        request_states();
        {
            int touched = 0;
#pragma unroll 4
            for (int o = wave; o < kn; o += WPB) {
                const CONST_AS int *w = reinterpret_cast<const CONST_AS int *>(ops + (k + o));
                static_assert(sizeof(DevOp) > 192 && sizeof(DevOp) <= 256, "one read per 64 bytes of the descriptor");
                touched ^= w[0] ^ w[16] ^ w[32] ^ w[48] ^ w[sizeof(DevOp) / 4 - 1];
            }
            asm volatile("" ::"s"(touched));
        }
        [[maybe_unused]] unsigned long long c0a = T4_CLK();
        for (int o0 = 0; o0 < kn; o0 += 64) {
            const int on = kn - o0 < 64 ? kn - o0 : 64;
            if (o0 > 0) {
                lds_barrier();
                if (threadIdx.x == 0) s_npair = 0;
                lds_barrier();
            }
            for (int t = threadIdx.x; t < on; t += kTravWg) {
                const CONST_AS DevOp &d = ops[k + o0 + t];
                s_opi[t][0] = d.lds_left;
                s_opi[t][1] = d.lds_right;
                s_opi[t][2] = d.left_kind == CHILD_LEAF ? 1 : (d.left_kind == CHILD_PAIR ? 2 : 0);
                s_opi[t][3] = d.right_kind == CHILD_LEAF ? 1 : (d.right_kind == CHILD_PAIR ? 2 : 0);
                s_opl[t][0] = op_child_len(d, 0);
                s_opl[t][1] = op_child_len(d, 1);
#pragma unroll
                for (int q = 0; q < 4; q++) s_opl[t][2 + q] = d.pair_len[q];
                if (d.left_kind == CHILD_PAIR) s_pair[atomicAdd(&s_npair, 1)] = 2 * t;
                if (d.right_kind == CHILD_PAIR) s_pair[atomicAdd(&s_npair, 1)] = 2 * t + 1;
            }
            lds_barrier();
            for (int t = threadIdx.x; t < on * 2 * B; t += kTravWg) {
                const int o = t / (2 * B), r = t - o * (2 * B), child = r / B, e = r - child * B;
                s_reg[s_opi[o][child] + e] = exp(s_model[16 + (e & 3)] * (s_model[20 + (e >> 2)] * s_opl[o][child]));
            }
            const int np = s_npair;
            for (int t = threadIdx.x; t < np * 2 * B; t += kTravWg) {
                const int pi = t / (2 * B), r = t - pi * (2 * B), w = r / B, e = r - w * B, o = s_pair[pi] >> 1, child = s_pair[pi] & 1;
                s_reg[s_opi[o][child] + (1 + kPairRows + 6 * w) * B + e] =
                    exp(s_model[16 + (e & 3)] * (s_model[20 + (e >> 2)] * s_opl[o][2 + 2 * child + w]));
            }
            lds_barrier();
            c0a = T4_CLK();
            auto leaf_table = [&](double *reg, int e) {
                const int c = e >> 2, x = e & 3;
                const LeafE4 E = leaf_e4(s_model + x * 4, reg + c * 4);
#pragma unroll
                for (int row = 0; row < 4; row++) reg[B + row * B + e] = E.entry(s_tip + row * 4);
                reg[B + 4 * B + e] = 1.0;
            };
            for (int t = threadIdx.x; t < on * 2 * B; t += kTravWg) {
                const int o = t / (2 * B), r = t - o * (2 * B), child = r / B, e = r - child * B;
                if (s_opi[o][2 + child] == 1) leaf_table(s_reg + s_opi[o][child], e);
            }
            if (np == 0) continue;
            for (int t = threadIdx.x; t < np * 2 * B; t += kTravWg) {
                const int pi = t / (2 * B), r = t - pi * (2 * B), w = r / B, e = r - w * B, o = s_pair[pi] >> 1, child = s_pair[pi] & 1;
                leaf_table(s_reg + s_opi[o][child] + (1 + kPairRows + 6 * w) * B, e);
            }
            lds_barrier();
#pragma unroll 1
            for (int t = threadIdx.x; t < np * C * kPairRows; t += kTravWg) {
                const int pi = t / (C * kPairRows), q = t - pi * (C * kPairRows), c = q / kPairRows, code = q - c * kPairRows;
                const int o = s_pair[pi] >> 1, child = s_pair[pi] & 1, sa = code / 5, sb = code - 5 * sa;
                double *reg = s_reg + s_opi[o][child];
                const double *ta = reg + (2 + kPairRows + sa) * B + c * 4, *tb = reg + (8 + kPairRows + sb) * B + c * 4;
                double tmp[4], l[4];
#pragma unroll
                for (int x = 0; x < 4; x++) tmp[x] = __dmul_rn(ta[x], tb[x]);
#pragma unroll
                for (int i = 0; i < 4; i++) {
                    double v = __dmul_rn(uinv[i * 4], tmp[0]);
                    v = fma(uinv[i * 4 + 1], tmp[1], v);
                    v = fma(uinv[i * 4 + 2], tmp[2], v);
                    v = fma(uinv[i * 4 + 3], tmp[3], v);
                    l[i] = __dmul_rn(reg[c * 4 + i], v);
                }
#pragma unroll
                for (int x = 0; x < 4; x++) {
                    double v = __dmul_rn(U[x * 4], l[0]);
                    v = fma(U[x * 4 + 1], l[1], v);
                    v = fma(U[x * 4 + 2], l[2], v);
                    reg[B + code * B + c * 4 + x] = fma(U[x * 4 + 3], l[3], v);
                }
            }
        }
        [[maybe_unused]] const unsigned long long c0b = T4_CLK();
        if constexpr (SP == 1) {
            asm volatile("s_waitcnt vmcnt(0)" ::: "memory");
        } else
        if (active) {
            for (int o0 = 0; o0 < kn; o0 += 16) {
                uint8_t vl[16], vr[16];
#pragma unroll
                for (int j = 0; j < 16; j++) {
                    const CONST_AS DevOp *d = ops + (k + (o0 + j < kn ? o0 + j : kn - 1));
                    vl[j] = *(d->sl + poff);
                    vr[j] = *(d->sr + poff);
                }
#pragma unroll
                for (int j = 0; j < 16; j++) {
                    if (o0 + j < kn) {
                        const CONST_AS DevOp *d = ops + (k + o0 + j);
                        w_states[d->sl_slot * 64 + lane] = vl[j];
                        w_states[d->sr_slot * 64 + lane] = vr[j];
                    }
                }
            }
        }
        __syncthreads();
        if (!active) { k += kn; continue; }
#ifdef IQHIP_T4_TRACE
        { const unsigned long long cz = T4_CLK(); t4_fill += cz - c0; t4_f1 += c0a - c0; t4_f2 += c0b - c0a; }
#endif

        for (int kk = 0; kk < kn; kk++, k++) {
            [[maybe_unused]] const unsigned long long c1 = T4_CLK();
            const CONST_AS DevOp *op = ops + k;
            const bool pairL = op->left_kind == CHILD_PAIR, pairR = op->right_kind == CHILD_PAIR;
            const bool leafL = op->left_kind == CHILD_LEAF || pairL;
            const bool holdL = op->left_kind == CHILD_HOLD;
            const bool leafR = op->right_kind == CHILD_LEAF || pairR;
            const bool tip_tip = leafL && leafR && !pairL && !pairR;
            const int pair_row_l = op->pair_row_l, pair_row_r = op->pair_row_r;
            int16_t *const dst_sc_p = op->dst_sc;
            const int out_row = op->out_row, rule = op->no_scale, push_hold = op->push_hold;
            int sc = 0;
            const int sL = w_states[op->sl_slot * 64 + lane];
            const int sR = w_states[op->sr_slot * 64 + lane];
            if (!leafL) sc += holdL ? hold_sc : pf_sc;
            if (HAS_LOAD && op->right_kind == CHILD_LOAD) {
                load_vec4_off<CL>(op->ld, voff, prev);
                prev_sc = *reinterpret_cast<const int16_t *>(reinterpret_cast<const char *>(op->ld_sc) + soff);
            }
            if (!leafR) sc += prev_sc;
            const CONST_AS DevOp *nx = ops + (k + 1);
            const int nreal = nx->real_mask;
            const char *nx_pf = (nreal & 1) ? reinterpret_cast<const char *>(nx->pf) + voff : nullptr;
            if (nreal & 1) pf_sc = *reinterpret_cast<const int16_t *>(reinterpret_cast<const char *>(nx->pf_sc) + soff);
            char *dstp = reinterpret_cast<char *>(op->dst) + voff;
            [[maybe_unused]] const unsigned long long c2 = T4_CLK();
            double lh_max = node_update4<CL, C>(leafL, holdL, leafR, pairL, pairR, s_reg + op->lds_left, s_reg + op->lds_right,
                                                s_tip, U, uinv, sL, sR, A.state_unknown, nx_pf, dstp, coff, PF, HOLD, prev);
            if (SP == 2) lh_max = fmax(lh_max, __shfl_xor(lh_max, 32, 64));
            [[maybe_unused]] const unsigned long long c3 = T4_CLK() + (lh_max == -1.0 ? 1 : 0);
            const ScaleChoice ch = scale_choice(rule, tip_tip, lh_max, invar);
            double my_scale = 0.0;
            const unsigned long long any = __ballot(ch.scale);
            if (__builtin_expect(any != 0, 0)) {
                if (ch.scale) {
                    if (ch.zero) {
#pragma unroll
                        for (int e = 0; e < BL; e++) prev[e] = s_tip[A.state_unknown * 4 + (e & 3)];
                    } else {
#pragma unroll
                        for (int e = 0; e < BL; e++) prev[e] *= kScalingThresholdInv;
                    }
                    sc += ch.events();
                    my_scale = (lead && ptn < A.nptn) ? ch.events() * (kLogScalingThreshold * freq) : 0.0;
#ifndef IQHIP_ABLATE_NOSTORE
                    store_vec4_off<CL>(op->dst, voff, prev);
#endif
                }
            }
            prev_sc = sc;
            if (push_hold) {
#pragma unroll
                for (int e = 0; e < BL; e++) HOLD[e] = prev[e];
                hold_sc = sc;
            }
#ifndef IQHIP_ABLATE_NOSTORE
            if (SP == 1 || lead) *reinterpret_cast<int16_t *>(reinterpret_cast<char *>(dst_sc_p) + soff) = (int16_t)sc;
#endif
            double ws = 0.0;
            if (any) ws = wave_sum(my_scale);
            if (lane == 0) {
                fold_store(&A.slab[(size_t)(2 + out_row) * A.nwaves + gw], ws);
                if (any) fold_flag(A.fold, 2 + out_row);
                if (pair_row_l >= 0) fold_store(&A.slab[(size_t)(2 + pair_row_l) * A.nwaves + gw], 0.0);
                if (pair_row_r >= 0) fold_store(&A.slab[(size_t)(2 + pair_row_r) * A.nwaves + gw], 0.0);
            }
#ifdef IQHIP_T4_TRACE
            { const unsigned long long c4 = T4_CLK(); t4_head += c2 - c1; t4_upd += c3 - c2; t4_tail += c4 - c3; t4_n++; }
#endif
        }
    }
#ifdef IQHIP_T4_TRACE
    if (t4_on) {
        atomicAdd(&g_t4[0], t4_fill); atomicAdd(&g_t4[1], t4_head); atomicAdd(&g_t4[2], t4_upd); atomicAdd(&g_t4[3], t4_tail);
        atomicAdd(&g_t4[4], t4_n); atomicAdd(&g_t4[5], 1ull); atomicAdd(&g_t4[6], t4_f1); atomicAdd(&g_t4[7], t4_f2);
    }
#endif
// ... 27 lines not shown
        }
        if (SP == 2) lh += __shfl_xor(lh, 32, 64);
        double pc = 0.0;
        if (A.nobs < A.nptn) {
            if (lead && ptn >= A.nobs && ptn < A.nptn) {
                int ssc = (A.root.b_kind == CHILD_PREV) ? prev_sc : (int)A.root.b_sc[ptn];
                if (A.root.a_kind != CHILD_LEAF) ssc += (A.root.a_kind == CHILD_PREV) ? prev_sc : (int)A.root.a_sc[ptn];
                pc = (ssc >= 1 ? lh * kScalingThreshold : lh) + invar;
            }
        }
        lh += invar;
        const double plh = log(fabs(lh));
        if (SP == 1 || lead) A.pattern_lh[ptn] = plh;
        const double acc = (lead && ptn < A.nobs) ? plh * freq : 0.0;
        const double ws = wave_sum(acc);
        const double wpc = (A.nobs < A.nptn) ? wave_sum(pc) : 0.0;
        if (lane == 0) {
            fold_store(&A.slab[gw], ws);
            fold_store(&A.slab[(size_t)A.nwaves + gw], wpc);
        }
    }
    if (A.fold.enabled) fold_tail(A.fold);
}

template <int C, bool HAS_LOAD, int SP>
static hipError_t launch_trav(iqhip_engine *e, Trav4Args &A) {
    const size_t lds = trav4_lds_bytes(4 * C, e->plan.lds_doubles, e->plan.state_slots);
    (void)raise_lds_ceiling<&k_traverse4<C, HAS_LOAD, SP>>(e, kTrav4MaxLdsBytes);
    A.ngroups = trav4_ngroups(e);
    hipLaunchKernelGGL((k_traverse4<C, HAS_LOAD, SP>), dim3((unsigned)(A.ngroups * A.nsegs_launch)), dim3(kTravWg), lds, e->stream, A);
    return hipGetLastError();
}

template <int C>
static hipError_t launch_trav_c(iqhip_engine *e, Trav4Args &A) {
    if constexpr (C % 2 == 0) {
        if (e->lane_split == 2) return A.has_load ? launch_trav<C, true, 2>(e, A) : launch_trav<C, false, 2>(e, A);
    }
    return A.has_load ? launch_trav<C, true, 1>(e, A) : launch_trav<C, false, 1>(e, A);
}

hipError_t launch_traverse4(iqhip_engine *e, const int *seg_table, int nsegs, bool has_load, const DevBranch *root, int nwaves,
                            int fold_rows) {
#ifdef IQHIP_T4_TRACE
    {
        static int calls = 0;
        if (++calls % 100 == 0) {
            unsigned long long h[8];
            (void)hipDeviceSynchronize();
            (void)hipMemcpyFromSymbol(h, HIP_SYMBOL(g_t4), sizeof h);
            if (h[4]) fprintf(stderr, "[t4] waves %llu ops %llu: per op head %.0f update %.0f tail %.0f clk; chunk fills %.0f clk per wave (exponentials %.0f, tables %.0f)\n",
                              h[5], h[4], (double)h[1] / h[4], (double)h[2] / h[4], (double)h[3] / h[4], (double)h[0] / h[5], (double)h[6] / h[5], (double)h[7] / h[5]);
            unsigned long long z[8] = {0, 0, 0, 0, 0, 0, 0, 0};
            (void)hipMemcpyToSymbol(HIP_SYMBOL(g_t4), z, sizeof z);
        }
    }
#endif
    Trav4Args A;
    A.fold.slab = e->d_slab.p;
    A.fold.result = e->d_result;
    A.fold.ticket = e->d_fold_ticket.p;
    A.fold.flags = e->d_fold_flags.p;
    A.fold.nwaves = nwaves;
    A.fold.nrows_scale = fold_rows > 0 ? fold_rows : 0;
    A.fold.root_rows = root ? (e->n_unobs > 0 ? 2 : 1) : 0;
    A.fold.enabled = fold_rows >= 0 ? 1 : 0;
    A.fold.done = nullptr;
    A.fold.seq = 0;
    if (A.fold.enabled && e->poll_result && e->d_result == e->d_result_own) {
        A.fold.seq = ++e->result_seq;
        A.fold.done = e->d_done;
        e->poll_pending = true;
        e->folded_rows = A.fold.nrows_scale;
    }
    A.ops = e->d_ops.p;
    A.evec = e->d_evec;
    A.inv_evec = e->d_inv_evec;
    A.tip = e->d_tip;
    A.freq = e->d_freq.p;
    A.invar = e->d_invar.p;
    A.eval = e->d_eval;
    A.rates = e->d_rates;
    A.props = e->d_props;
    A.pattern_lh = e->d_pattern_lh.p;
    A.slab = e->d_slab.p;
    A.ntiles = e->ntiles;
    A.nptn = e->nptn;
    A.nobs = e->nptn - e->n_unobs;
    A.segs = seg_table;
    A.nsegs_launch = nsegs;
    A.has_load = has_load ? 1 : 0;
    A.nwaves = nwaves;
    A.state_unknown = e->state_unknown;
    A.has_root = root ? 1 : 0;
    A.lds_reg_doubles = e->plan.lds_doubles;
    A.state_slots = e->plan.state_slots;
    if (root) A.root = *root; else A.root = DevBranch{nullptr, nullptr, nullptr, nullptr, nullptr, 0, 0, 0.0};
    A.small_plan = 0;
    A.small_segs[0] = A.small_segs[1] = 0;
    if (e->plan.small && nsegs == 1) {
        A.small_plan = 1;
        A.small_segs[1] = e->plan.small_nops;
        for (int q = 0; q < kSmallPlanOps; q++) A.small_ops[q] = e->h_ops.p[q];
    } else {
        for (int q = 0; q < kSmallPlanOps; q++) A.small_ops[q] = DevOp{};
    }
    switch (e->ncat) {
        case 1: return launch_trav_c<1>(e, A);
        case 2: return launch_trav_c<2>(e, A);
        case 3: return launch_trav_c<3>(e, A);
        case 4: return launch_trav_c<4>(e, A);
        case 5: return launch_trav_c<5>(e, A);
        case 6: return launch_trav_c<6>(e, A);
        case 7: return launch_trav_c<7>(e, A);
        case 8: return launch_trav_c<8>(e, A);
        default: return hipErrorInvalidValue;
    }
}

template <int C>
__global__ __launch_bounds__(256) void k_theta4(DevBranch br, const double *__restrict__ tip,
                                                int state_unknown, double *__restrict__ theta,
                                                int64_t ntiles) {
    constexpr int B = 4 * C;
    __shared__ double s_tip[32 * 4];
    for (int t = threadIdx.x; t < (state_unknown + 1) * 4; t += 256) s_tip[t] = tip[t];
    __syncthreads();
    const int lane = threadIdx.x & 63;
    const int64_t tile = (int64_t)blockIdx.x * 4 + (threadIdx.x >> 6);
    if (tile >= ntiles) return;
    const int64_t ptn = tile * 64 + lane;
    double Bv[B], Th[B];
    load_vec4<C>(br.b, tile, lane, Bv);
    if (br.a_kind == CHILD_LEAF) {
        const int s = br.a_states[ptn];
#pragma unroll
        for (int e = 0; e < B; e++) Th[e] = s_tip[s * 4 + (e & 3)] * Bv[e];
    } else {
        double Av[B];
        load_vec4<C>(br.a, tile, lane, Av);
#pragma unroll
        for (int e = 0; e < B; e++) Th[e] = Av[e] * Bv[e];
    }
    store_vec4<C>(theta, tile, lane, Th);
}

hipError_t launch_theta4(iqhip_engine *e, const DevBranch &br, double *theta_out) {
    const int grid = (int)((e->ntiles + 3) / 4);
    double *const theta = theta_out ? theta_out : e->d_theta.p;
#define IQ_THETA(Cv)                                                                        \
    case Cv:                                                                                \
        hipLaunchKernelGGL(k_theta4<Cv>, dim3(grid), dim3(256), 0, e->stream, br, e->d_tip, \
                           e->state_unknown, theta, e->ntiles);                          \
        break;
    switch (e->ncat) {
        IQ_THETA(1) IQ_THETA(2) IQ_THETA(3) IQ_THETA(4) IQ_THETA(5) IQ_THETA(6) IQ_THETA(7) IQ_THETA(8)
        default: return hipErrorInvalidValue;
    }
#undef IQ_THETA
    return hipGetLastError();
}

template <int C, int MODE>
__global__ __launch_bounds__(256) void k_theta_reduce4(
    const double *__restrict__ theta, const double *__restrict__ eval,
    const double *__restrict__ rates, const double *__restrict__ props, double len,
    const double *__restrict__ freq, const double *__restrict__ invar,
    double *__restrict__ pattern_lh, double *__restrict__ slab, int64_t ntiles, int64_t nptn,
    int nwaves, int64_t nobs, const int16_t *__restrict__ a_sc, const int16_t *__restrict__ b_sc,
    const NewtonState *st, size_t theta_stride, int task_rows, const int16_t *const *task_sc) {
    constexpr int B = 4 * C;
    __shared__ double s_v0[B], s_v1[B], s_v2[B];
    if (theta_stride) {
        theta += (size_t)blockIdx.y * theta_stride;
        slab += (size_t)task_rows * blockIdx.y * nwaves;
        st += blockIdx.y;
        if (task_sc) { a_sc = task_sc[2 * blockIdx.y]; b_sc = task_sc[2 * blockIdx.y + 1]; }
    }
    if (st) {
        if (MODE == 0) {
            if (st->done) return;
            len = st->rts;
        } else {
            len = st->result;
        }
    }
    if (threadIdx.x < B) {
        const int c = threadIdx.x >> 2, i = threadIdx.x & 3;
        const double cof = eval[i] * rates[c];
        const double v = exp(cof * len) * props[c];
        s_v0[threadIdx.x] = v;
        s_v1[threadIdx.x] = cof * v;
        s_v2[threadIdx.x] = cof * (cof * v);
    }
    __syncthreads();
    const int lane = threadIdx.x & 63;
    const int64_t tile = (int64_t)blockIdx.x * 4 + (threadIdx.x >> 6);
    if (tile >= ntiles) return;
    const int gw = (int)tile;
    const int64_t ptn = tile * 64 + lane;
    double Th[B];
    load_vec4<C>(theta, tile, lane, Th);
    const double f = (ptn < nobs) ? freq[ptn] : 0.0;
// ... 207 lines not shown
```

### iq-tree_amd/csrc/plan.hip

```cpp
#include <math.h>
#include <stdio.h>
#include <stdlib.h>
#include <string.h>

#include <algorithm>
#include <unordered_set>

#include "iqhip_internal.h"

using namespace iqhip;

namespace {

int fail(int code, const std::string &msg) { return set_error(code, msg); }
constexpr int kSentinels = 2;

int devops_for(size_t bytes) { return (int)((bytes + sizeof(DevOp) - 1) / sizeof(DevOp)); }

struct Units {
    std::vector<int> order;
    std::vector<int> seg_of;
    std::vector<std::pair<int, int>> units;
    std::vector<int> stage_units;
    int top_begin = 0;
// ... 417 lines not shown
            }
            uses.push_back({k, side});
            use_slot.push_back(slot);
        }
    }
    const size_t need = (size_t)e->ntaxa + (size_t)noverflow;
    if (need > e->d_leaf_tab.cap / per) {
        HIPCHK(e->d_leaf_tab.ensure(e, (need + 16) * per));
        e->plan_cache.uploaded.clear();
        dirty.insert(dirty.end(), clean.begin(), clean.end());
        clean.clear();
        e->tab_len.assign(e->d_leaf_tab.cap / per, NAN);
    }
    if (e->tab_len.size() < e->d_leaf_tab.cap / per) e->tab_len.resize(e->d_leaf_tab.cap / per, NAN);
    for (int k = 0; k < nops; k++) e->h_ops.p[k].tabL = e->h_ops.p[k].tabR = e->d_leaf_tab.p;
    for (size_t q = 0; q < uses.size(); q++) {
        DevOp &d = e->h_ops.p[uses[q].first];
        (uses[q].second ? d.tabR : d.tabL) = e->d_leaf_tab.p + (size_t)use_slot[q] * per;
    }
    for (std::vector<TabJob> *v : {&dirty, &clean})
        for (TabJob &j : *v) {
            const size_t slot = (size_t)j.tab;
            j.tab = e->d_leaf_tab.p + slot * per;
            e->tab_len[slot] = slot < (size_t)e->ntaxa ? j.len : NAN;
            e->plan.tab_jobs.push_back(j);
        }
    e->plan.tab_dirty = (int)dirty.size();
    e->plan.nleaf_tabs = (int)e->plan.tab_jobs.size();
    return IQHIP_OK;
}

int assign_cherry_tables(iqhip_engine *e, int nops, const std::vector<int> &seg_of) {
    const bool have_pair = e->planner ? e->cherry_s2 > 0 : (e->pair && e->cherry_model_synced);
    if (!(cherry_candidate(e) && e->mfma_pipelined && have_pair && nops >= 8)) return IQHIP_OK;
    const size_t per = (size_t)e->cherry_npairs * e->block;
    const size_t want = (size_t)2 * e->ntaxa + 16;
    const bool fresh = e->d_cherry_tab.cap < want * per;
    if (fresh) HIPCHK(e->d_cherry_tab.ensure(e, want * per));
    const size_t cherry_cap = e->d_cherry_tab.cap / per;
    if (fresh || e->cherry_slots.size() + (size_t)e->ntaxa / 2 + 1 > cherry_cap) {
        e->cherry_slot_of.clear();
        e->cherry_slots.clear();
    }
    const uint64_t stamp = ++e->cherry_stamp;
    for (int k = 0; k < nops; k++) {
        DevOp &d = e->h_ops.p[k];
        if (d.left_kind != CHILD_LEAF || d.right_kind != CHILD_LEAF || d.left_len_p || d.right_len_p) continue;
        if ((top_stage_may_share_tiles(e) || top_stage_may_mix_roles64(e)) && seg_of[k] == 0) continue;
        const uint64_t tl = (uint64_t)((d.sl - e->d_states.p) / e->nptn_pad), tr = (uint64_t)((d.sr - e->d_states.p) / e->nptn_pad);
        const uint64_t key = (tl << 32) | tr;
        auto it = e->cherry_slot_of.find(key);
        int slot;
        if (it == e->cherry_slot_of.end()) {
            if (e->cherry_slots.size() >= cherry_cap) continue;
            slot = (int)e->cherry_slots.size();
            e->cherry_slots.emplace_back();
            e->cherry_slot_of[key] = slot;
        } else {
            slot = it->second;
        }
        iqhip_engine::CherrySlot &cs = e->cherry_slots[slot];
        const bool same = cs.len_l == d.left_len && cs.len_r == d.right_len;
        if (cs.stamp == stamp && !same) continue;
        if (!same || cs.model_version != e->model_version) {
            cs.len_l = d.left_len;
            cs.len_r = d.right_len;
            cs.model_version = 0;
            if (cs.stamp != stamp) e->plan.cherry_jobs.push_back(slot);
        }
        cs.stamp = stamp;
        d.cherry = e->d_cherry_tab.p + (size_t)slot * per;
        e->plan.uses_cherry = true;
    }
    return IQHIP_OK;
}

int lay_out_lds(iqhip_engine *e, int nops, const std::vector<int> &seg_of) {
    const int B = e->block, budget = lds_budget(e);
    const bool tables_in_lds = e->mfma && e->mfma_pipelined && e->n == 20 && e->plan.nleaf_tabs > 0;
    const int leaf_sz = (!e->mfma || e->wide4) ? child_region_blocks(CHILD_LEAF) * B : (tables_in_lds ? (int)leaf_table_doubles(e) : B);
    const int pair_sz = child_region_blocks(CHILD_PAIR) * B;
    const int slot_sz = e->mfma ? 0 : trav4_lds(B).slot_doubles;
    int chunk_start = 0, used = slot_sz, regs = 0, max_used = 0, slots = 1, max_slots = 1;
    for (int k = 0; k < nops; k++) {
        DevOp &d = e->h_ops.p[k];
        const int szl = d.left_kind == CHILD_LEAF ? leaf_sz : (d.left_kind == CHILD_PAIR ? pair_sz : B);
        const int szr = d.right_kind == CHILD_LEAF ? leaf_sz : (d.right_kind == CHILD_PAIR ? pair_sz : B);
        const int nleaf = child_is_table(d.left_kind) + child_is_table(d.right_kind);
        const int need = szl + szr + nleaf * slot_sz;
        if (slot_sz + need > budget) return fail(IQHIP_ERR_UNSUPPORTED, "nstates*ncat too large for the LDS plan regions");
        const bool rows_full = !e->mfma && slots + nleaf > kTrav4RowSlots;
        if ((used + need > budget || rows_full || seg_of[k] != seg_of[k - (k > 0)]) && k > chunk_start) {
            e->h_ops.p[chunk_start].chunk_nops = k - chunk_start;
            e->h_ops.p[chunk_start].chunk_slots = slots;
            chunk_start = k; used = slot_sz; regs = 0; slots = 1;
        }
        d.lds_left = regs; d.lds_right = regs + szl;
        regs += szl + szr;
        used += need;
        if (regs > max_used) max_used = regs;
        d.sl_slot = child_is_table(d.left_kind) ? slots++ : 0;
        d.sr_slot = child_is_table(d.right_kind) ? slots++ : 0;
        if (slots > max_slots) max_slots = slots;
    }
    if (nops > 0) {
        e->h_ops.p[chunk_start].chunk_nops = nops - chunk_start;
        e->h_ops.p[chunk_start].chunk_slots = slots;
    }
    e->plan.state_slots = max_slots;
    e->plan.lds_doubles = max_used;
    return IQHIP_OK;
}

int check_plan(iqhip_engine *e, int nops, int nsentinels) {
    std::unordered_set<const void *> vecs, scs;
    for (const Slab &sl : e->slabs) { vecs.insert(sl.plh.p); scs.insert(sl.sc.p); }
    vecs.insert(e->dummy.plh.p);
    scs.insert(e->dummy.sc.p);
    const size_t per = (e->mfma && e->mfma_pipelined) ? leaf_table_doubles(e) : 0;
    char msg[256];
    auto bad = [&](int k, const char *what) {
        snprintf(msg, sizeof msg, "plan check: op %d of %d (+%d sentinels): %s", k, nops, nsentinels, what);
        return fail(IQHIP_ERR_INVALID, msg);
    };
    auto state_row = [&](const uint8_t *p) {
        if (!p || !e->d_states.p || p < e->d_states.p) return false;
        const size_t off = (size_t)(p - e->d_states.p);
        return off % (size_t)e->nptn_pad == 0 && off / (size_t)e->nptn_pad < (size_t)e->ntaxa;
    };
    auto pair_row = [&](const uint8_t *p) {
        if (!p || !e->d_pair_rows.p || p < e->d_pair_rows.p) return false;
        const size_t off = (size_t)(p - e->d_pair_rows.p);
        return off % (size_t)e->nptn_pad == 0 && off / (size_t)e->nptn_pad < e->pair_row_of.size();
    };
    auto table = [&](const double *p) {
        if (e->plan.nleaf_tabs == 0 && !e->d_leaf_tab.p) return p == nullptr;
        if (!p || !e->d_leaf_tab.p || p < e->d_leaf_tab.p || per == 0) return false;
        const size_t off = (size_t)(p - e->d_leaf_tab.p);
        return off % per == 0 && off / per < e->d_leaf_tab.cap / per;
    };
    for (int k = 0; k < nops + nsentinels; k++) {
        const DevOp &d = e->h_ops.p[k];
        if (!vecs.count(d.dst) || d.dst == nullptr) return bad(k, "dst is not a vector slab");
        if (!scs.count(d.dst_sc)) return bad(k, "dst_sc is not a counter slab");
        if (!vecs.count(d.pf)) return bad(k, "pf (streamed child) is not a vector slab / the dummy slab");
        if (!scs.count(d.pf_sc)) return bad(k, "pf_sc is not a counter slab / the dummy");
        if (!vecs.count(d.ld)) return bad(k, "ld (second memory child) is not a vector slab / the dummy slab");
        if (!scs.count(d.ld_sc)) return bad(k, "ld_sc is not a counter slab / the dummy");
        const bool pl = k < nops && d.left_kind == CHILD_PAIR, pr = k < nops && d.right_kind == CHILD_PAIR;
        if ((pl || pr) && (e->mfma || e->wide4)) return bad(k, "pair child in a plan of another kernel than k_traverse4");
        if (!(pl ? pair_row(d.sl) : state_row(d.sl)) || !(pr ? pair_row(d.sr) : state_row(d.sr)))
            return bad(k, "sl / sr is not a row of the state matrix (a pair-code row for a pair child, and only for one)");
        if ((pl && !(d.pair_len[0] >= 0.0 && d.pair_len[1] >= 0.0)) || (pr && !(d.pair_len[2] >= 0.0 && d.pair_len[3] >= 0.0)))
            return bad(k, "pair child with a negative or NaN pendant branch length");
        if ((pl != (d.pair_row_l >= 0)) || (pr != (d.pair_row_r >= 0)) || d.pair_row_l >= e->plan.nrows || d.pair_row_r >= e->plan.nrows)
            return bad(k, "pair_row is not the row of a removed op");
        if (!table(d.tabL) || !table(d.tabR)) return bad(k, "tabL / tabR is not a K2 table slot");
        if (d.cherry) {
            const size_t cper = (size_t)e->cherry_npairs * e->block;
            if (!e->d_cherry_tab.p || cper == 0 || d.cherry < e->d_cherry_tab.p || (size_t)(d.cherry - e->d_cherry_tab.p) % cper != 0 ||
                (size_t)(d.cherry - e->d_cherry_tab.p) / cper >= e->d_cherry_tab.cap / cper || k >= nops || d.left_kind != CHILD_LEAF ||
                d.right_kind != CHILD_LEAF)
                return bad(k, "cherry is not a cherry-table slot of an op with two leaf children");
        }
        if (k >= nops) continue;
        if (d.dst == e->dummy.plh.p || d.dst_sc == e->dummy.sc.p) return bad(k, "a real op writes the dummy slab");
        const bool lk = d.left_kind == CHILD_LEAF || d.left_kind == CHILD_PAIR || d.left_kind == CHILD_PF || d.left_kind == CHILD_HOLD ||
                        (d.left_kind == CHILD_LOAD && e->mfma && !e->mfma_pipelined);
        const bool rk = d.right_kind == CHILD_LEAF || d.right_kind == CHILD_PAIR || d.right_kind == CHILD_PREV || d.right_kind == CHILD_LOAD;
        if (!lk || !rk) return bad(k, "child kinds are not in canonical form");
        if (d.left_kind == CHILD_PF && (d.pf == e->dummy.plh.p || !(d.real_mask & 1))) return bad(k, "streamed child without a real vector");
        if (d.left_kind != CHILD_PF && !(e->mfma && !e->mfma_pipelined) && (d.real_mask & 1)) return bad(k, "real_mask set without a streamed child");
        if (d.right_kind == CHILD_LOAD && d.ld == e->dummy.plh.p) return bad(k, "second memory child without a real vector");
        if (d.dst == d.pf || d.dst == d.ld) return bad(k, "op writes one of its own children");
        if (!(d.left_len >= 0.0) || !(d.right_len >= 0.0)) return bad(k, "negative or NaN branch length");
        if (d.out_row < 0 || d.out_row >= e->plan.nrows) return bad(k, "out_row outside the caller's op list");
        if (d.lds_left < 0 || d.lds_right < 0 || d.lds_left > e->plan.lds_doubles || d.lds_right > e->plan.lds_doubles)
            return bad(k, "LDS region outside the launch's allocation");
        if (d.sl_slot < 0 || d.sr_slot < 0 || d.sl_slot >= e->plan.state_slots || d.sr_slot >= e->plan.state_slots)
            return bad(k, "leaf-state slot outside the launch's allocation");
        if (d.chunk_nops < 0 || k + d.chunk_nops > nops) return bad(k, "LDS chunk runs past the plan");
        if (e->wide4) {
            if ((d.left_kind != CHILD_LEAF && d.left_kind != CHILD_LOAD) || (d.right_kind != CHILD_LEAF && d.right_kind != CHILD_LOAD))
                return bad(k, "wide 4-state op is not in the (memory, memory) form");
            if ((d.left_kind == CHILD_LOAD && d.pf == e->dummy.plh.p) || (d.right_kind == CHILD_LOAD && d.ld == e->dummy.plh.p))
                return bad(k, "memory child without a real vector");
            const int szl = (d.left_kind == CHILD_LEAF ? 6 : 1) * e->block, szr = (d.right_kind == CHILD_LEAF ? 6 : 1) * e->block;
            if (d.lds_left + szl > e->plan.lds_doubles || d.lds_right + szr > e->plan.lds_doubles ||
                (d.lds_left < d.lds_right + szr && d.lds_right < d.lds_left + szl))
                return bad(k, "LDS regions of the two children overlap or leave the launch's allocation");
            if (d.no_scale < 0 || d.no_scale > 2) return bad(k, "unknown scaling rule");
        }
    }
    for (int k = 0; k < nops;) {
        const DevOp &c = e->h_ops.p[k];
        if (c.chunk_nops <= 0) return bad(k, "op is not covered by an LDS chunk");
        if (!e->mfma) {
            int next = 1, regs = 0;
            for (int q = k; q < k + c.chunk_nops; q++) {
                const DevOp &d = e->h_ops.p[q];
                if (d.sl_slot != (child_is_table(d.left_kind) ? next : 0)) return bad(q, "leaf-state slots of the chunk are not 1 .. n in op order");
                next += child_is_table(d.left_kind);
                if (d.sr_slot != (child_is_table(d.right_kind) ? next : 0)) return bad(q, "leaf-state slots of the chunk are not 1 .. n in op order");
                next += child_is_table(d.right_kind);
                const int szl = child_region_blocks(d.left_kind) * e->block, szr = child_region_blocks(d.right_kind) * e->block;
                if (d.lds_left < d.lds_right + szr && d.lds_right < d.lds_left + szl) return bad(q, "LDS regions of the two children overlap");
                regs = std::max(regs, std::max(d.lds_left + szl, d.lds_right + szr));
            }
            if (c.chunk_slots != next) return bad(k, "chunk_slots is not the chunk's slot count");
            if (next > kTrav4RowSlots) return bad(k, "more leaf-state slots than the kernel's row-pointer list holds");
            if (next > e->plan.state_slots || regs > e->plan.lds_doubles) return bad(k, "LDS chunk outside the launch's allocation");
            if (regs + next * trav4_lds(e->block).slot_doubles > lds_budget(e)) return bad(k, "LDS chunk over the LDS budget");
        }
        k += c.chunk_nops;
    }
    const int *tab = reinterpret_cast<const int *>(e->h_ops.p + e->plan.table_off);
    int covered = 0;
    for (int u = 0; u <= e->plan.nunits; u++) {
        const int b = tab[2 * u], n = tab[2 * u + 1];
        if (b < 0 || n < 0 || b + n > nops) return bad(b, "segment outside the plan");
        covered += n;
    }
    if (covered != nops) return bad(nops, "segments do not cover the plan exactly once");
    return IQHIP_OK;
}

int upload_plan(iqhip_engine *e, size_t nbytes) {
    if (e->planner) return IQHIP_OK;
    std::vector<char> &up = e->plan_cache.uploaded;
    const char *h = reinterpret_cast<const char *>(e->h_ops.p);
    if (e->plan.small) {
    } else if (up.size() == nbytes && memcmp(up.data(), h, nbytes) == 0) {
        return IQHIP_OK;
    } else if (e->plan_arena_on && e->plan_arena_used + nbytes <= e->h_plan_arena.cap) {
        char *slice = e->h_plan_arena.p + e->plan_arena_used;
        memcpy(slice, h, nbytes);
        e->plan_arena_used += (nbytes + 255) / 256 * 256;
        HIPCHK(hipMemcpyAsync(e->d_ops.p, slice, nbytes, hipMemcpyHostToDevice, e->stream));
    } else {
        HIPCHK(hipMemcpyAsync(e->d_ops.p, e->h_ops.p, nbytes, hipMemcpyHostToDevice, e->stream));
        HIPCHK(hipEventRecord(e->staging_free, e->stream));
        e->staging_busy = true;
    }
    up.assign(h, h + nbytes);
    return IQHIP_OK;
}

int finish_and_upload(iqhip_engine *e, int nops, const iqhip_node_op *ops_in, int nops_in, Units &u, const std::vector<int> *explicit_segs,
                      const double *const *len_ptrs, int last_dst) {
    Plan &p = e->plan;
    for (int q = 0; q < kSentinels; q++) dummy_op(e, e->h_ops.p[nops + q]);
    p.table_off = nops + kSentinels;
    const int table_ops = segment_table_ops(u);
    int *tab = reinterpret_cast<int *>(e->h_ops.p + p.table_off);
    memset(tab, 0, sizeof(DevOp) * (size_t)table_ops);
    tab[0] = u.top_begin; tab[1] = nops - u.top_begin;
    for (size_t i = 0; i < u.units.size(); i++) { tab[2 + 2 * i] = u.units[i].first; tab[3 + 2 * i] = u.units[i].second; }
    p.nunits = (int)u.units.size();
    p.stage_units = std::move(u.stage_units);
    p.top_nops = nops - u.top_begin;
    p.jobs_off = p.table_off + table_ops;
    const int jobs_ops = devops_for(sizeof(TabJob) * p.tab_jobs.size());
    if (jobs_ops > 0) {
        memset(e->h_ops.p + p.jobs_off, 0, sizeof(DevOp) * (size_t)jobs_ops);
        memcpy(e->h_ops.p + p.jobs_off, p.tab_jobs.data(), sizeof(TabJob) * p.tab_jobs.size());
    }
    PlanCache &c = e->plan_cache;
    c.ops_in.assign((const char *)ops_in, (const char *)(ops_in + nops_in));
    c.segs = explicit_segs ? *explicit_segs : std::vector<int>();
    c.version = len_ptrs ? 0 : e->keymap_version;
    c.dst = last_dst;
    p.small = e->small_plans && kernel_takes_small_plan(e) && !explicit_segs && u.units.empty() && nops > 0 && nops + kSentinels <= kSmallPlanOps;
    p.small_nops = nops;
    if (e->planner && nops > 0) {
        const std::string &br = e->debug_break_plan;
        if (br == "tab") e->h_ops.p[nops - 1].tabL = nullptr;
        else if (br == "sentinel") e->h_ops.p[nops + kSentinels - 1].pf = nullptr;
        else if (br == "states") e->h_ops.p[0].sr = nullptr;
        else if (br == "pair_row") {
            for (int k = 0; k < nops; k++)
                if (e->h_ops.p[k].left_kind == CHILD_LEAF && !e->pair_row_of.empty()) { e->h_ops.p[k].sl = e->d_pair_rows.p; break; }
        } else if (br == "pair_region") {
            for (int k = 0; k < nops; k++)
                if (e->h_ops.p[k].left_kind == CHILD_PAIR) {
                    e->h_ops.p[k].lds_left = lds_budget(e);
                    e->plan.lds_doubles = lds_budget(e) + child_region_blocks(CHILD_PAIR) * e->block;
                    break;
                }
        }
        else if (br == "cherry")
            for (int k = 0; k < nops; k++)
                if (e->h_ops.p[k].cherry) { e->h_ops.p[k].cherry += 8; break; }
    }
    if (e->check_plans) {
        const int rc = check_plan(e, nops, kSentinels);
        if (rc) { c.invalidate(); return rc; }
    }
    return upload_plan(e, sizeof(DevOp) * (size_t)(p.jobs_off + jobs_ops));
}

}

namespace iqhip {

int resolve_child(iqhip_engine *e, uint64_t key, int32_t leaf, int prev_dst, const double **plh, const int16_t **sc,
                  const uint8_t **states, int32_t *kind) {
    *plh = nullptr; *sc = nullptr; *states = nullptr;
    if (leaf >= 0) {
        if (leaf >= e->ntaxa) return fail(IQHIP_ERR_INVALID, "leaf id out of range");
        *states = e->d_states.p + (size_t)leaf * e->nptn_pad;
        *kind = CHILD_LEAF;
        return IQHIP_OK;
    }
    int idx;
    int rc = slab_for_key(e, key, false, &idx);
    if (rc) return rc;
    *plh = e->slabs[idx].plh.p;
    *sc = e->slabs[idx].sc.p;
    *kind = (idx == prev_dst) ? CHILD_PREV : CHILD_LOAD;
    return IQHIP_OK;
}

int build_branch(iqhip_engine *e, iqhip_branch_end a, iqhip_branch_end b, double len, int prev_dst, DevBranch *br) {
    if (!(len >= 0.0)) return fail(IQHIP_ERR_INVALID, "negative or NaN branch length");
    if (a.leaf >= 0 && b.leaf >= 0)
        return fail(IQHIP_ERR_INVALID, "branch with two leaf ends (2-taxon tree) is not supported");
    if (b.leaf >= 0) std::swap(a, b);
    const uint8_t *st_unused;
    int rc = resolve_child(e, a.key, a.leaf, prev_dst, &br->a, &br->a_sc, &br->a_states, &br->a_kind);
    if (rc) return rc;
    rc = resolve_child(e, b.key, b.leaf, prev_dst, &br->b, &br->b_sc, &st_unused, &br->b_kind);
    if (rc) return rc;
    br->len = len;
    return IQHIP_OK;
}

bool leaf_tables_follow_model(iqhip_engine *e) {
    if (e->tab_model_version == e->model_version) return false;
    std::fill(e->tab_len.begin(), e->tab_len.end(), NAN);
    const size_t per = leaf_table_doubles(e);
    for (const TabJob &j : e->plan.tab_jobs) {
        const size_t slot = (size_t)(j.tab - e->d_leaf_tab.p) / per;
        if (slot < (size_t)e->ntaxa) e->tab_len[slot] = j.len;
    }
    e->tab_model_version = e->model_version;
    return true;
}

constexpr int kRows64BudgetSlack = 128;

int lds_budget(const iqhip_engine *e) {
    const int B = e->block, nx = e->state_unknown + 1 - e->n;
    if (!e->mfma) return e->lds_budget_bytes / 8 - trav4_lds(B).s_reg;
    if (e->wide4) {
        const int kb = e->mfma_lds_kb >= 0 ? e->mfma_lds_kb : kWide4LdsKb;
        return kb * 1024 / 8 - std::max(wide4_lds(e->nclass, B).sReg, generic_lds(4, nx).sReg);
    }
    int fixed = !e->mfma_pipelined ? generic_lds(e->n, nx).sReg
                : e->row_split     ? rows64_lds(nx).sReg + kRows64BudgetSlack
                                   : mfma2_lds(e->n, nx).sReg;
    if (e->mfma_pipelined && e->n == 64) fixed = std::max(fixed, rows64_lds(nx).sReg + kRows64BudgetSlack);
    const int total_kb = e->mfma_lds_kb >= 0 ? e->mfma_lds_kb : (e->n == 20 ? 75 : 78);
    if (e->plan.nhold > 0) fixed += mfma2_park_doubles(B);
    int budget = (total_kb * 1024) / 8 - fixed;
    if (e->mfma_lds_kb < 0 && !e->mfma_pipelined && budget < 2 * B) budget = kTravMaxLdsBytes / 8 - fixed;
    return budget;
}

TravLaunch choose_traverse_mfma(const iqhip_engine *e, bool top_stage, int nsegs) {
    const int n = e->n, C = e->ncat, nx = e->state_unknown + 1 - n, regs = e->plan.lds_doubles;
    const int64_t tiles = e->ntiles;
    TravLaunch L = {TRAV_NONE, false, 0, 0, 0, 0, -1};
    int fixed = 0, waves_per_tile = 1;
    if (!e->mfma_pipelined) {
        if (e->wide4 && !e->wide4_generic) {
            L.variant = TRAV_WIDE4;
            fixed = wide4_lds(e->nclass, e->block).sReg;
        } else if (n == 20) {
            L.variant = e->mix_split ? TRAV_MIX20_SPLIT : TRAV_MIX20;
            waves_per_tile = e->mix_split ? 4 : 1;
            fixed = mix20_lds().sReg;
        } else if (n == 64 || n == 4) {
            L.variant = TRAV_GENERIC;
            fixed = generic_lds(n, nx).sReg;
        }
    } else if ((n == 20 && (C == 4 || C == 1)) || (n == 64 && C == 1)) {
        L.tab = e->plan.nleaf_tabs > 0 || e->leaf_tables;
        L.variant = TRAV_M2;
        fixed = mfma2_lds(n, nx).sReg;
        if (n == 64) {
            const int64_t per_round = (int64_t)e->num_cus * 4, rounds = tiles / per_round, rest = tiles - rounds * per_round;
            if (e->row_split) {
                L.variant = TRAV_ROWS64;
                waves_per_tile = 4;
                fixed = rows64_lds(nx).sReg;
            } else if (top_stage && nsegs == 1 && top_stage_may_mix_roles64(e) && rounds >= 1 && rest > 0 && rest <= per_round / 2) {
                L.variant = TRAV_TOP64;
                L.nfull = (int)(rounds * e->num_cus);
                L.ngroups = (int)(tiles - (int64_t)L.nfull * 4);
                fixed = top64_fixed_doubles(nx);
            }
        } else if (C == 4 && e->cat_split) {
            L.variant = TRAV_M2_CAT_SPLIT;
            waves_per_tile = 4;
        } else if (C == 4 && !L.tab && top_stage && top_stage_may_share_tiles(e)) {
            const int64_t per_round = (int64_t)e->num_cus * 3 * 2, rounds = tiles / per_round, rest = tiles - rounds * per_round;
            L.variant = TRAV_M2_TOP_CS2;
            waves_per_tile = 2;
            if (e->mixed_top && nsegs == 1 && rounds >= 1 && rest > 0 && rest <= per_round / 4) {
                L.variant = TRAV_TOP20;
                L.nfull = (int)(rounds * e->num_cus * 3);
                L.ngroups = (int)(tiles - (int64_t)L.nfull * 2);
            }
        }
    }
    if (L.variant == TRAV_NONE) return L;
    if (L.nfull > 0) L.grid = L.nfull + L.ngroups;
    else {
        L.ngroups = (int)((tiles * waves_per_tile + kTravWg / 64 - 1) / (kTravWg / 64));
        L.grid = L.ngroups * nsegs;
    }
    L.lds_bytes = (size_t)(fixed + regs) * sizeof(double);
    if (L.variant == TRAV_M2 && n < 64 && e->plan.nhold > 0) {
        L.hold_off = fixed + regs;
        L.lds_bytes += (size_t)mfma2_park_doubles(e->block) * sizeof(double);
    }
    return L;
}

int build_plan(iqhip_engine *e, const iqhip_node_op *ops, int nops, int *last_dst, const std::vector<int> *explicit_segs,
               const double *const *len_ptrs) {
    if (nops + 2 > e->result_cap) return fail(IQHIP_ERR_INVALID, "too many node updates in one submission");
    if (plan_is_cached(e, ops, nops, explicit_segs, len_ptrs)) {
        *last_dst = e->plan_cache.dst;
        mark_virtual_slabs(e);
        return IQHIP_OK;
    }
    e->plan_cache.version = 0;
    if (e->staging_busy) {
        HIPCHK(hipEventSynchronize(e->staging_free));
        e->staging_busy = false;
    }
    e->plan = Plan();
    e->plan.cherry_model = e->model_version;
    e->plan.nrows = nops;
    const iqhip_node_op *const ops_in = ops;
    const int nops_in = nops;
    Kept kept;
    bool removed = false;
    int rc = select_pair_children(e, ops, nops, explicit_segs, len_ptrs, kept, &removed);
    if (rc) return rc;
    if (removed) { ops = kept.ops.data(); nops = (int)kept.ops.size(); }
    Units u;
    rc = cut_units(e, ops, nops, explicit_segs, u);
    if (!rc) rc = ensure_plan_capacity(e, nops + kSentinels + segment_table_ops(u) + devops_for(sizeof(TabJob) * (size_t)(2 * nops + 1)));
    if (!rc) rc = fill_descriptors(e, ops, nops, u, len_ptrs, last_dst, removed ? &kept : nullptr);
    if (!rc) park_operands(e, nops, u.seg_of);
    if (!rc) rc = assign_leaf_tables(e, nops);
    if (!rc) rc = assign_cherry_tables(e, nops, u.seg_of);
    if (!rc) rc = lay_out_lds(e, nops, u.seg_of);
    if (!rc) rc = finish_and_upload(e, nops, ops_in, nops_in, u, explicit_segs, len_ptrs, *last_dst);
    if (!rc) mark_virtual_slabs(e);
    return rc;
}

}
```

### iq-tree_amd/csrc/trav_phases.h

```cpp
#pragma once
#include "iqhip_internal.h"
namespace iqhip {
struct ScaleChoice {
    bool zero, scale;
    __device__ __forceinline__ int events() const { return zero ? 4 : 1; }
};
template <typename KEY>
__device__ __forceinline__ ScaleChoice scale_choice_on(int rule, bool tip_tip, KEY max, double invar, KEY threshold) {
    const bool zero = rule == 2 && !tip_tip && max == KEY(0);
    const bool do_scale = zero || (!tip_tip && (max < threshold) && (invar == 0.0) && rule != 1);
    return {zero, do_scale};
}
__device__ __forceinline__ ScaleChoice scale_choice(int rule, bool tip_tip, unsigned lmax, double invar) {
    return scale_choice_on<unsigned>(rule, tip_tip, lmax, invar, kScalingThresholdHi);
}
__device__ __forceinline__ ScaleChoice scale_choice(int rule, bool tip_tip, double lh_max, double invar) {
    return scale_choice_on<double>(rule, tip_tip, lh_max, invar, kScalingThreshold);
}
__device__ __forceinline__ unsigned promote_nonzero(int rule, unsigned nz, unsigned lmax) {
    return (rule == 2 && nz != 0 && lmax == 0) ? 1u : lmax;
}
template <int CS, int W>
__device__ __forceinline__ unsigned tile_max(unsigned (&s)[2][W][16], int par, int wave, int p, int g, unsigned lmax) {
    if (g == 0) s[par][wave][p] = lmax;
    __syncthreads();
    const int w0 = (wave / CS) * CS;
    if constexpr (CS == 4) return max(max(s[par][w0][p], s[par][w0 + 1][p]), max(s[par][w0 + 2][p], s[par][w0 + 3][p]));
#pragma unroll
    for (int q = 0; q < CS; q++) lmax = max(lmax, s[par][w0 + q][p]);
    return lmax;
}
__device__ __forceinline__ void post_scale_sum(double *slab, int *fold_flags, int out_row, int nwaves, int64_t tl, bool writer,
                                               double my_scale) {
    const double ws = __any(my_scale != 0.0) ? wave_sum64(my_scale) : 0.0;
    if (!writer) return;
    slab[(size_t)(2 + out_row) * nwaves + (int)tl] = ws;
    if (ws != 0.0) __hip_atomic_fetch_or(&fold_flags[2 + out_row], 1, __ATOMIC_RELAXED, __HIP_MEMORY_SCOPE_AGENT);
}
struct FillAll { template <typename Op> __device__ __forceinline__ bool operator()(const Op &, int) const { return false; } };
template <int WG, typename Ops, class Ev, class Rate, class Skip>
__device__ __forceinline__ void fill_exponentials(Ops ops, int k, int kn, int B, double *sReg, Ev ev, Rate rate, Skip skip) {
    for (int t = threadIdx.x; t < kn * 2 * B; t += WG) {
        const int o = t / (2 * B), r = t - o * (2 * B), child = r / B, e = r - child * B;
        const auto &d = ops[k + o];
        if (skip(d, child)) continue;
        sReg[(child ? d.lds_right : d.lds_left) + e] = exp(ev(e) * (rate(e) * op_child_len(d, child)));
    }
}
struct LeafE4 {
    double e0, e1, e2, e3;
    __device__ __forceinline__ double entry(const double *tip4) const {
        return __dadd_rn(__dadd_rn(__dmul_rn(e0, tip4[0]), __dmul_rn(e1, tip4[1])), __dadd_rn(__dmul_rn(e2, tip4[2]), __dmul_rn(e3, tip4[3])));
    }
};
__device__ __forceinline__ LeafE4 leaf_e4(const double *Urow, const double *ex4) {
    return {__dmul_rn(Urow[0], ex4[0]), __dmul_rn(Urow[1], ex4[1]), __dmul_rn(Urow[2], ex4[2]), __dmul_rn(Urow[3], ex4[3])};
}
__device__ __forceinline__ double leaf_entry4(const double *Urow, const double *ex4, const double *tip4) {
    return leaf_e4(Urow, ex4).entry(tip4);
}
}
```

Baseline: 35000 M updates/s.

## Precompute per-plan LDS fill image once and bulk-load it into LDS

Adds a global-memory 'fill image' holding each chunk's exponentials, leaf tables and pair rows, built by a new kernel only when the plan or model version changes. The traversal kernel then copies the chunk's image into LDS with global_load_lds instead of recomputing exp and table entries in every workgroup. This is meant to remove redundant transcendental and table arithmetic repeated across all pattern tiles. In exchange it costs extra device memory, an extra kernel launch on rebuilds, and cache-invalidation logic tied to model_version and the plan cache. It also adds debug entry points to inspect the image.

```diff
diff --git a/include/iqhip.h b/include/iqhip.h
--- a/include/iqhip.h
+++ b/include/iqhip.h
@@ -296,6 +296,11 @@
 int iqhip_debug_planner_plain_taxa(iqhip_engine *e, const uint8_t *plain);
 int iqhip_debug_plan_removed(iqhip_engine *e, int32_t *out, int nrows);
 
+int iqhip_debug_fill_image(iqhip_engine *e, int64_t *built, int64_t *reused, int64_t *bytes);
+int iqhip_debug_plan_submit(iqhip_engine *e, const iqhip_node_op *ops, int nops, const int32_t *segs, int nsegs, int device_lengths);
+int iqhip_debug_planner_event(iqhip_engine *e, int what);
+int iqhip_debug_fill_image_chunks(iqhip_engine *e, int64_t *out, int cap, int *nchunks);
+
 void iqhip_debug_memory(int64_t *device_bytes, int64_t *host_bytes);
 void iqhip_debug_fail_alloc(int nth);
 
diff --git a/iq-tree_amd/__init__.py b/iq-tree_amd/__init__.py
--- a/iq-tree_amd/__init__.py
+++ b/iq-tree_amd/__init__.py
@@ -25,7 +25,8 @@
     "iqhip_comm_size", "iqhip_update_partials_async", "iqhip_lnl_from_theta_async",
     "iqhip_newton_host_init", "iqhip_newton_host_update", "iqhip_newton_host_result",
     "iqhip_debug_create_planner", "iqhip_debug_plan", "iqhip_timing_plan_bytes", "iqhip_timing_collective_read", "iqhip_optimize_sweep", "iqhip_debug_cherry_tables",
-    "iqhip_debug_path_counts", "iqhip_debug_plan_shape", "iqhip_debug_plan_layout", "iqhip_debug_pair_children", "iqhip_debug_pair_rows", "iqhip_debug_planner_plain_taxa", "iqhip_debug_plan_removed", "iqhip_debug_memory", "iqhip_debug_fail_alloc",
+    "iqhip_debug_path_counts", "iqhip_debug_plan_shape", "iqhip_debug_plan_layout", "iqhip_debug_pair_children", "iqhip_debug_pair_rows", "iqhip_debug_planner_plain_taxa", "iqhip_debug_plan_removed",
+    "iqhip_debug_fill_image", "iqhip_debug_plan_submit", "iqhip_debug_planner_event", "iqhip_debug_fill_image_chunks", "iqhip_debug_memory", "iqhip_debug_fail_alloc",
     "iqhip_ptnlh_reserve", "iqhip_ptnlh_put_current", "iqhip_ptnlh_fetch", "iqhip_optimize_branch_batch_rows",
     "iqhip_branch_tests", "iqhip_ptnlh_rell",
     "iqhip_ptnlh_upload", "iqhip_gen_boot_samples", "iqhip_ptnlh_diff_variance", "iqhip_tree_tests", "iqhip_multiscale_bp",
@@ -211,6 +212,10 @@
     lib.iqhip_debug_plan_shape.argtypes = [vp, C.POINTER(C.c_int64), C.c_int]
     lib.iqhip_debug_plan_layout.argtypes = [vp, C.POINTER(C.c_int32), C.c_int]
     lib.iqhip_debug_pair_rows.argtypes = [vp, C.POINTER(C.c_int64), C.POINTER(C.c_int64), C.POINTER(C.c_int64)]
+    lib.iqhip_debug_fill_image.argtypes = [vp, C.POINTER(C.c_int64), C.POINTER(C.c_int64), C.POINTER(C.c_int64)]
+    lib.iqhip_debug_plan_submit.argtypes = [vp, C.POINTER(NodeOp), C.c_int, C.POINTER(C.c_int32), C.c_int, C.c_int]
+    lib.iqhip_debug_planner_event.argtypes = [vp, C.c_int]
+    lib.iqhip_debug_fill_image_chunks.argtypes = [vp, C.POINTER(C.c_int64), C.c_int, C.POINTER(C.c_int)]
     lib.iqhip_debug_memory.argtypes = [C.POINTER(C.c_int64), C.POINTER(C.c_int64)]
     lib.iqhip_debug_memory.restype = None
     lib.iqhip_debug_fail_alloc.argtypes = [C.c_int]
diff --git a/iq-tree_amd/csrc/engine.hip b/iq-tree_amd/csrc/engine.hip
--- a/iq-tree_amd/csrc/engine.hip
+++ b/iq-tree_amd/csrc/engine.hip
@@ -574,6 +574,7 @@
         rc = iqhip_create(&e->pair, e->device, e->n, e->ncat, npairs, 2);
         if (rc) return rc;
         e->pair->cherry_on = false;
+        e->pair->fill_image.on = false;
         e->pair->check_plans = e->check_plans;
         rc = iqhip_set_stream(e->pair, e->stream);
         if (rc) return rc;
@@ -766,6 +767,8 @@
     if (e->plan.uses_cherry)
         for (int k = 0; k < nops; k++) e->cherry_ops_total += e->h_ops.p[k].cherry != nullptr;
     timing_begin(e);
+    rc = fill_image_submission(e);
+    if (rc) return rc;
     const int *table = reinterpret_cast<const int *>(e->d_ops.p + e->plan.table_off);
     {
         int off = 2;
@@ -1022,6 +1025,15 @@
     return IQHIP_OK;
 }
 
+extern "C" int iqhip_debug_fill_image(iqhip_engine *e, int64_t *built, int64_t *reused, int64_t *bytes) {
+    if (!e) return fail(IQHIP_ERR_INVALID, "null engine");
+    if (!e->shards.empty()) e = e->shards[0];
+    if (built) *built = e->fill_image.built;
+    if (reused) *reused = e->fill_image.reused;
+    if (bytes) *bytes = (e->plan.image_ok && !e->plan.small) ? e->plan.image_doubles * (int64_t)sizeof(double) : 0;
+    return IQHIP_OK;
+}
+
 extern "C" int iqhip_debug_planner_plain_taxa(iqhip_engine *e, const uint8_t *plain) {
     if (!e || !e->planner) return fail(IQHIP_ERR_INVALID, "iqhip_debug_planner_plain_taxa needs a planning-only engine");
     e->taxon_plain.clear();
@@ -1355,9 +1367,19 @@
 
 extern "C" int iqhip_debug_plan(iqhip_engine *e, const iqhip_node_op *ops, int nops) {
     if (!e || !e->planner) return fail(IQHIP_ERR_INVALID, "iqhip_debug_plan needs a planning-only engine");
-    if (nops < 0 || (nops > 0 && !ops)) return fail(IQHIP_ERR_INVALID, "bad ops array");
+    return iqhip_debug_plan_submit(e, ops, nops, nullptr, 0, 0);
+}
+
+extern "C" int iqhip_debug_plan_submit(iqhip_engine *e, const iqhip_node_op *ops, int nops, const int32_t *segs, int nsegs,
+                                       int device_lengths) {
+    if (!e || !e->planner) return fail(IQHIP_ERR_INVALID, "iqhip_debug_plan_submit needs a planning-only engine");
+    if (nops < 0 || (nops > 0 && !ops) || nsegs < 0 || (nsegs > 0 && !segs)) return fail(IQHIP_ERR_INVALID, "bad ops array");
     int last_dst = -1;
-    const int rc = build_plan(e, ops, nops, &last_dst, nullptr);
+    const std::vector<int> seg_list(segs, segs + nsegs);
+    std::vector<const double *> lp;
+    if (device_lengths) lp.assign((size_t)2 * nops, e->dummy.plh.p);
+    int rc = build_plan(e, ops, nops, &last_dst, nsegs > 0 ? &seg_list : nullptr, device_lengths ? lp.data() : nullptr);
+    if (!rc) rc = fill_image_submission(e);
     if (!rc) {
         e->cherry_built_total += (int64_t)e->plan.cherry_jobs.size();
         for (int slot : e->plan.cherry_jobs) e->cherry_slots[slot].model_version = e->model_version;
@@ -1365,6 +1387,29 @@
         for (int k = 0; k < nops; k++) e->cherry_ops_total += e->h_ops.p[k].cherry != nullptr;
     }
     return rc;
+}
+
+extern "C" int iqhip_debug_planner_event(iqhip_engine *e, int what) {
+    if (!e || !e->planner || what < 0 || what > 1) return fail(IQHIP_ERR_INVALID, "iqhip_debug_planner_event needs a planning-only engine and event 0 or 1");
+    if (what == 0) e->model_version++;
+    else { e->pair_row_of.clear(); e->plan_cache.invalidate(); }
+    return IQHIP_OK;
+}
+
+extern "C" int iqhip_debug_fill_image_chunks(iqhip_engine *e, int64_t *out, int cap, int *nchunks) {
+    if (!e || !e->planner || !nchunks || (cap > 0 && !out)) return fail(IQHIP_ERR_INVALID, "iqhip_debug_fill_image_chunks needs a planning-only engine");
+    int n = 0;
+    for (int k = 0; k < e->plan.small_nops && !e->mfma; k += e->h_ops.p[k].chunk_nops, n++) {
+        int regs = 0;
+        for (int q = k; q < k + e->h_ops.p[k].chunk_nops; q++) {
+            const DevOp &d = e->h_ops.p[q];
+            regs = std::max(regs, std::max(d.lds_left + child_region_blocks(d.left_kind) * e->block,
+                                           d.lds_right + child_region_blocks(d.right_kind) * e->block));
+        }
+        if (n < cap) { out[2 * n] = (int64_t)e->h_ops.p[k].image_off * 8; out[2 * n + 1] = (int64_t)regs * 8; }
+    }
+    *nchunks = n;
+    return IQHIP_OK;
 }
 
 extern "C" int iqhip_debug_plan_shape(iqhip_engine *e, int64_t *out, int n) {
diff --git a/iq-tree_amd/csrc/iqhip_internal.h b/iq-tree_amd/csrc/iqhip_internal.h
--- a/iq-tree_amd/csrc/iqhip_internal.h
+++ b/iq-tree_amd/csrc/iqhip_internal.h
@@ -57,7 +57,7 @@
     const double *right_len_p;
     const double *cherry;
     int32_t chunk_slots;
-    int32_t _pad_slots;
+    int32_t image_off;
     double pair_len[4];
     int32_t pair_row_l, pair_row_r;
 };
@@ -178,6 +178,8 @@
     struct Virtual { int slab; int32_t taxon_l, taxon_r; double len_l, len_r; };
     std::vector<Virtual> virt;
     int nrows = 0;
+    int64_t image_doubles = 0;
+    bool image_ok = false;
 };
 
 struct PlanCache {
@@ -570,6 +572,13 @@
     int64_t pair_ops_removed = 0, pair_slabs_expanded = 0;
     int64_t pair_row_restarts = 0, pair_ops_without_row = 0;
 
+    struct FillImage {
+        iqhip::DevBuf<double> buf;
+        uint64_t model = 0;
+        bool on = true, plan_hit = false, use = false;
+        int64_t built = 0, reused = 0;
+    } fill_image;
+
     std::unordered_map<uint64_t, int> key2slab;
     std::vector<iqhip::Slab> slabs;
     std::vector<int> free_slabs;
@@ -777,6 +786,8 @@
 int expand_virtual_slabs(iqhip_engine *e);
 hipError_t launch_pair_expand(iqhip_engine *e, const Slab &s);
 hipError_t launch_pair_codes(iqhip_engine *e, const uint8_t *row_l, const uint8_t *row_r, uint8_t *out);
+int fill_image_submission(iqhip_engine *e);
+hipError_t launch_fill4_image(iqhip_engine *e, int nops);
 bool cherry_candidate(const iqhip_engine *e);
 
 int build_plan(iqhip_engine *e, const iqhip_node_op *ops, int nops, int *last_dst,
diff --git a/iq-tree_amd/csrc/kernels_valu4.hip b/iq-tree_amd/csrc/kernels_valu4.hip
--- a/iq-tree_amd/csrc/kernels_valu4.hip
+++ b/iq-tree_amd/csrc/kernels_valu4.hip
@@ -40,6 +40,7 @@
     const double *eval;
     const double *rates;
     const double *props;
+    const double *image;
     double *pattern_lh;
     double *slab;
     int64_t ntiles;
@@ -314,79 +315,68 @@
             asm volatile("" ::"s"(touched));
         }
         [[maybe_unused]] unsigned long long c0a = T4_CLK();
-        for (int o0 = 0; o0 < kn; o0 += 64) {
-            const int on = kn - o0 < 64 ? kn - o0 : 64;
-            if (o0 > 0) {
+        if (A.image != nullptr) {
+            const int ioff = ops[k].image_off;
+            int ebytes = (ops[k + kn].image_off - ioff) * 8;
+            ebytes = ebytes < A.lds_reg_doubles * 8 ? ebytes : A.lds_reg_doubles * 8;
+            const char *const src = reinterpret_cast<const char *>(A.image + ioff);
+            uint32_t tx = threadIdx.x;
+            asm volatile("" : "+v"(tx));
+            const uint32_t l16 = (tx & 63u) * 16u;
+            for (int p = wave * 1024; p < ebytes; p += WPB * 1024) {
+                if (p + (int)l16 < ebytes)
+                    __builtin_amdgcn_global_load_lds((const __attribute__((address_space(1))) void *)(src + p + l16),
+                                                     (__attribute__((address_space(3))) void *)(reinterpret_cast<char *>(s_reg) + p), 16, 0, 0);
+            }
+        } else {
+            for (int o0 = 0; o0 < kn; o0 += 64) {
+                const int on = kn - o0 < 64 ? kn - o0 : 64;
+                if (o0 > 0) {
+                    lds_barrier();
+                    if (threadIdx.x == 0) s_npair = 0;
+                    lds_barrier();
+                }
+                for (int t = threadIdx.x; t < on; t += kTravWg) {
+                    const CONST_AS DevOp &d = ops[k + o0 + t];
+                    s_opi[t][0] = d.lds_left;
+                    s_opi[t][1] = d.lds_right;
+                    s_opi[t][2] = d.left_kind == CHILD_LEAF ? 1 : (d.left_kind == CHILD_PAIR ? 2 : 0);
+                    s_opi[t][3] = d.right_kind == CHILD_LEAF ? 1 : (d.right_kind == CHILD_PAIR ? 2 : 0);
+                    s_opl[t][0] = op_child_len(d, 0);
+                    s_opl[t][1] = op_child_len(d, 1);
+    #pragma unroll
+                    for (int q = 0; q < 4; q++) s_opl[t][2 + q] = d.pair_len[q];
+                    if (d.left_kind == CHILD_PAIR) s_pair[atomicAdd(&s_npair, 1)] = 2 * t;
+                    if (d.right_kind == CHILD_PAIR) s_pair[atomicAdd(&s_npair, 1)] = 2 * t + 1;
+                }
                 lds_barrier();
-                if (threadIdx.x == 0) s_npair = 0;
+                for (int t = threadIdx.x; t < on * 2 * B; t += kTravWg) {
+                    const int o = t / (2 * B), r = t - o * (2 * B), child = r / B, e = r - child * B;
+                    s_reg[s_opi[o][child] + e] = fill4_exp(s_model, e, s_opl[o][child]);
+                }
+                const int np = s_npair;
+                for (int t = threadIdx.x; t < np * 2 * B; t += kTravWg) {
+                    const int pi = t / (2 * B), r = t - pi * (2 * B), w = r / B, e = r - w * B, o = s_pair[pi] >> 1, child = s_pair[pi] & 1;
+                    s_reg[s_opi[o][child] + (1 + kPairRows + 6 * w) * B + e] = fill4_exp(s_model, e, s_opl[o][2 + 2 * child + w]);
+                }
                 lds_barrier();
-            }
-            for (int t = threadIdx.x; t < on; t += kTravWg) {
-                const CONST_AS DevOp &d = ops[k + o0 + t];
-                s_opi[t][0] = d.lds_left;
-                s_opi[t][1] = d.lds_right;
-                s_opi[t][2] = d.left_kind == CHILD_LEAF ? 1 : (d.left_kind == CHILD_PAIR ? 2 : 0);
-                s_opi[t][3] = d.right_kind == CHILD_LEAF ? 1 : (d.right_kind == CHILD_PAIR ? 2 : 0);
-                s_opl[t][0] = op_child_len(d, 0);
-                s_opl[t][1] = op_child_len(d, 1);
-#pragma unroll
-                for (int q = 0; q < 4; q++) s_opl[t][2 + q] = d.pair_len[q];
-                if (d.left_kind == CHILD_PAIR) s_pair[atomicAdd(&s_npair, 1)] = 2 * t;
-                if (d.right_kind == CHILD_PAIR) s_pair[atomicAdd(&s_npair, 1)] = 2 * t + 1;
-            }
-            lds_barrier();
-            for (int t = threadIdx.x; t < on * 2 * B; t += kTravWg) {
-                const int o = t / (2 * B), r = t - o * (2 * B), child = r / B, e = r - child * B;
-                s_reg[s_opi[o][child] + e] = exp(s_model[16 + (e & 3)] * (s_model[20 + (e >> 2)] * s_opl[o][child]));
-            }
-            const int np = s_npair;
-            for (int t = threadIdx.x; t < np * 2 * B; t += kTravWg) {
-                const int pi = t / (2 * B), r = t - pi * (2 * B), w = r / B, e = r - w * B, o = s_pair[pi] >> 1, child = s_pair[pi] & 1;
-                s_reg[s_opi[o][child] + (1 + kPairRows + 6 * w) * B + e] =
-                    exp(s_model[16 + (e & 3)] * (s_model[20 + (e >> 2)] * s_opl[o][2 + 2 * child + w]));
-            }
-            lds_barrier();
-            c0a = T4_CLK();
-            auto leaf_table = [&](double *reg, int e) {
-                const int c = e >> 2, x = e & 3;
-                const LeafE4 E = leaf_e4(s_model + x * 4, reg + c * 4);
-#pragma unroll
-                for (int row = 0; row < 4; row++) reg[B + row * B + e] = E.entry(s_tip + row * 4);
-                reg[B + 4 * B + e] = 1.0;
-            };
-            for (int t = threadIdx.x; t < on * 2 * B; t += kTravWg) {
-                const int o = t / (2 * B), r = t - o * (2 * B), child = r / B, e = r - child * B;
-                if (s_opi[o][2 + child] == 1) leaf_table(s_reg + s_opi[o][child], e);
-            }
-            if (np == 0) continue;
-            for (int t = threadIdx.x; t < np * 2 * B; t += kTravWg) {
-                const int pi = t / (2 * B), r = t - pi * (2 * B), w = r / B, e = r - w * B, o = s_pair[pi] >> 1, child = s_pair[pi] & 1;
-                leaf_table(s_reg + s_opi[o][child] + (1 + kPairRows + 6 * w) * B, e);
-            }
-            lds_barrier();
-#pragma unroll 1
-            for (int t = threadIdx.x; t < np * C * kPairRows; t += kTravWg) {
-                const int pi = t / (C * kPairRows), q = t - pi * (C * kPairRows), c = q / kPairRows, code = q - c * kPairRows;
-                const int o = s_pair[pi] >> 1, child = s_pair[pi] & 1, sa = code / 5, sb = code - 5 * sa;
-                double *reg = s_reg + s_opi[o][child];
-                const double *ta = reg + (2 + kPairRows + sa) * B + c * 4, *tb = reg + (8 + kPairRows + sb) * B + c * 4;
-                double tmp[4], l[4];
-#pragma unroll
-                for (int x = 0; x < 4; x++) tmp[x] = __dmul_rn(ta[x], tb[x]);
-#pragma unroll
-                for (int i = 0; i < 4; i++) {
-                    double v = __dmul_rn(uinv[i * 4], tmp[0]);
-                    v = fma(uinv[i * 4 + 1], tmp[1], v);
-                    v = fma(uinv[i * 4 + 2], tmp[2], v);
-                    v = fma(uinv[i * 4 + 3], tmp[3], v);
-                    l[i] = __dmul_rn(reg[c * 4 + i], v);
-                }
-#pragma unroll
-                for (int x = 0; x < 4; x++) {
-                    double v = __dmul_rn(U[x * 4], l[0]);
-                    v = fma(U[x * 4 + 1], l[1], v);
-                    v = fma(U[x * 4 + 2], l[2], v);
-                    reg[B + code * B + c * 4 + x] = fma(U[x * 4 + 3], l[3], v);
+                c0a = T4_CLK();
+                auto leaf_table = [&](double *reg, int e) { fill4_leaf_table(reg, B, e, s_model, s_tip); };
+                for (int t = threadIdx.x; t < on * 2 * B; t += kTravWg) {
+                    const int o = t / (2 * B), r = t - o * (2 * B), child = r / B, e = r - child * B;
+                    if (s_opi[o][2 + child] == 1) leaf_table(s_reg + s_opi[o][child], e);
+                }
+                if (np == 0) continue;
+                for (int t = threadIdx.x; t < np * 2 * B; t += kTravWg) {
+                    const int pi = t / (2 * B), r = t - pi * (2 * B), w = r / B, e = r - w * B, o = s_pair[pi] >> 1, child = s_pair[pi] & 1;
+                    leaf_table(s_reg + s_opi[o][child] + (1 + kPairRows + 6 * w) * B, e);
+                }
+                lds_barrier();
+    #pragma unroll 1
+                for (int t = threadIdx.x; t < np * C * kPairRows; t += kTravWg) {
+                    const int pi = t / (C * kPairRows), q = t - pi * (C * kPairRows), c = q / kPairRows, code = q - c * kPairRows;
+                    const int o = s_pair[pi] >> 1, child = s_pair[pi] & 1;
+                    fill4_pair_row(s_reg + s_opi[o][child], B, c, code, U, uinv);
                 }
             }
         }
@@ -413,6 +403,7 @@
                 }
             }
         }
+        if constexpr (SP == 2) asm volatile("s_waitcnt vmcnt(0)" ::: "memory");
         __syncthreads();
         if (!active) { k += kn; continue; }
 #ifdef IQHIP_T4_TRACE
@@ -606,6 +597,7 @@
     A.eval = e->d_eval;
     A.rates = e->d_rates;
     A.props = e->d_props;
+    A.image = e->fill_image.use ? e->fill_image.buf.p : nullptr;
     A.pattern_lh = e->d_pattern_lh.p;
     A.slab = e->d_slab.p;
     A.ntiles = e->ntiles;
@@ -643,6 +635,59 @@
 }
 
 template <int C>
+__global__ __launch_bounds__(64) void k_fill4_image(const DevOp *__restrict__ ops, const double *__restrict__ evec,
+                                                    const double *__restrict__ inv_evec, const double *__restrict__ eval,
+                                                    const double *__restrict__ rates, const double *__restrict__ tip,
+                                                    double *__restrict__ image) {
+    constexpr int B = 4 * C;
+    __shared__ double s_model[32], s_tip[16], s_r[child_region_blocks(CHILD_PAIR) * B];
+    const int t = threadIdx.x, child = blockIdx.x & 1;
+    const DevOp &d = ops[blockIdx.x >> 1];
+    const int kind = child ? d.right_kind : d.left_kind;
+    if (t < 20 + C) s_model[t] = t < 16 ? evec[t] : (t < 20 ? eval[t - 16] : rates[t - 20]);
+    if (t < 16) s_tip[t] = tip[t];
+    __syncthreads();
+    if (t < B) s_r[t] = fill4_exp(s_model, t, child ? d.right_len : d.left_len);
+    if (kind == CHILD_PAIR && t < 2 * B) {
+        const int w = t / B, e = t - w * B;
+        s_r[(1 + kPairRows + 6 * w) * B + e] = fill4_exp(s_model, e, d.pair_len[2 * child + w]);
+    }
+    __syncthreads();
+    if (kind == CHILD_LEAF && t < B) fill4_leaf_table(s_r, B, t, s_model, s_tip);
+    if (kind == CHILD_PAIR) {
+        if (t < 2 * B) {
+            const int w = t / B, e = t - w * B;
+            fill4_leaf_table(s_r + (1 + kPairRows + 6 * w) * B, B, e, s_model, s_tip);
+        }
+        __syncthreads();
+        const CONST_AS double *U = as_const(evec), *uinv = as_const(inv_evec);
+        for (int q = t; q < C * kPairRows; q += 64) {
+            const int c = q / kPairRows, code = q - c * kPairRows;
+            fill4_pair_row(s_r, B, c, code, U, uinv);
+        }
+    }
+    __syncthreads();
+    double *const out = image + d.image_off + (child ? d.lds_right : d.lds_left);
+    const int n = child_region_blocks(kind) * B;
+    for (int q = t; q < n; q += 64) out[q] = s_r[q];
+}
+
+hipError_t launch_fill4_image(iqhip_engine *e, int nops) {
+    if (nops <= 0) return hipSuccess;
+#define IQ_FI(Cv)                                                                                                         \
+    case Cv:                                                                                                              \
+        hipLaunchKernelGGL(k_fill4_image<Cv>, dim3((unsigned)(2 * nops)), dim3(64), 0, e->stream, e->d_ops.p, e->d_evec,  \
+                           e->d_inv_evec, e->d_eval, e->d_rates, e->d_tip, e->fill_image.buf.p);                          \
+        break;
+    switch (e->ncat) {
+        IQ_FI(1) IQ_FI(2) IQ_FI(3) IQ_FI(4) IQ_FI(5) IQ_FI(6) IQ_FI(7) IQ_FI(8)
+        default: return hipErrorInvalidValue;
+    }
+#undef IQ_FI
+    return hipGetLastError();
+}
+
+template <int C>
 __global__ __launch_bounds__(256) void k_theta4(DevBranch br, const double *__restrict__ tip,
                                                 int state_unknown, double *__restrict__ theta,
                                                 int64_t ntiles) {
diff --git a/iq-tree_amd/csrc/plan.hip b/iq-tree_amd/csrc/plan.hip
--- a/iq-tree_amd/csrc/plan.hip
+++ b/iq-tree_amd/csrc/plan.hip
@@ -523,8 +523,18 @@
     const int pair_sz = child_region_blocks(CHILD_PAIR) * B;
     const int slot_sz = e->mfma ? 0 : trav4_lds(B).slot_doubles;
     int chunk_start = 0, used = slot_sz, regs = 0, max_used = 0, slots = 1, max_slots = 1;
+    int64_t image = 0;
+    bool image_ok = !e->mfma && e->fill_image.on;
+    auto close_chunk = [&](int end) {
+        e->h_ops.p[chunk_start].chunk_nops = end - chunk_start;
+        e->h_ops.p[chunk_start].chunk_slots = slots;
+        if (e->mfma) return;
+        for (int q = chunk_start; q < end; q++) e->h_ops.p[q].image_off = (int32_t)image;
+        image += regs;
+    };
     for (int k = 0; k < nops; k++) {
         DevOp &d = e->h_ops.p[k];
+        if (d.left_len_p || d.right_len_p) image_ok = false;
         const int szl = d.left_kind == CHILD_LEAF ? leaf_sz : (d.left_kind == CHILD_PAIR ? pair_sz : B);
         const int szr = d.right_kind == CHILD_LEAF ? leaf_sz : (d.right_kind == CHILD_PAIR ? pair_sz : B);
         const int nleaf = child_is_table(d.left_kind) + child_is_table(d.right_kind);
@@ -532,8 +542,7 @@
         if (slot_sz + need > budget) return fail(IQHIP_ERR_UNSUPPORTED, "nstates*ncat too large for the LDS plan regions");
         const bool rows_full = !e->mfma && slots + nleaf > kTrav4RowSlots;
         if ((used + need > budget || rows_full || seg_of[k] != seg_of[k - (k > 0)]) && k > chunk_start) {
-            e->h_ops.p[chunk_start].chunk_nops = k - chunk_start;
-            e->h_ops.p[chunk_start].chunk_slots = slots;
+            close_chunk(k);
             chunk_start = k; used = slot_sz; regs = 0; slots = 1;
         }
         d.lds_left = regs; d.lds_right = regs + szl;
@@ -544,10 +553,10 @@
         d.sr_slot = child_is_table(d.right_kind) ? slots++ : 0;
         if (slots > max_slots) max_slots = slots;
     }
-    if (nops > 0) {
-        e->h_ops.p[chunk_start].chunk_nops = nops - chunk_start;
-        e->h_ops.p[chunk_start].chunk_slots = slots;
-    }
+    if (nops > 0) close_chunk(nops);
+    if (image * (int64_t)sizeof(double) > INT32_MAX) image_ok = false;
+    e->plan.image_doubles = image;
+    e->plan.image_ok = image_ok && image > 0;
     e->plan.state_slots = max_slots;
     e->plan.lds_doubles = max_used;
     return IQHIP_OK;
@@ -648,6 +657,10 @@
                 if (d.lds_left < d.lds_right + szr && d.lds_right < d.lds_left + szl) return bad(q, "LDS regions of the two children overlap");
                 regs = std::max(regs, std::max(d.lds_left + szl, d.lds_right + szr));
             }
+            for (int q = k; q < k + c.chunk_nops; q++)
+                if (e->h_ops.p[q].image_off != c.image_off) return bad(q, "image_off differs within a chunk");
+            if (c.image_off < 0 || c.image_off % 2 != 0 || (int64_t)c.image_off + regs > e->plan.image_doubles)
+                return bad(k, "the chunk's fill image is misaligned or outside the image");
             if (c.chunk_slots != next) return bad(k, "chunk_slots is not the chunk's slot count");
             if (next > kTrav4RowSlots) return bad(k, "more leaf-state slots than the kernel's row-pointer list holds");
             if (next > e->plan.state_slots || regs > e->plan.lds_doubles) return bad(k, "LDS chunk outside the launch's allocation");
@@ -667,9 +680,12 @@
 }
 
 int upload_plan(iqhip_engine *e, size_t nbytes) {
-    if (e->planner) return IQHIP_OK;
     std::vector<char> &up = e->plan_cache.uploaded;
     const char *h = reinterpret_cast<const char *>(e->h_ops.p);
+    if (e->planner) {
+        up.assign(h, h + nbytes);
+        return IQHIP_OK;
+    }
     if (e->plan.small) {
     } else if (up.size() == nbytes && memcmp(up.data(), h, nbytes) == 0) {
         return IQHIP_OK;
@@ -691,6 +707,7 @@
                       const double *const *len_ptrs, int last_dst) {
     Plan &p = e->plan;
     for (int q = 0; q < kSentinels; q++) dummy_op(e, e->h_ops.p[nops + q]);
+    e->h_ops.p[nops].image_off = (int32_t)p.image_doubles;
     p.table_off = nops + kSentinels;
     const int table_ops = segment_table_ops(u);
     int *tab = reinterpret_cast<int *>(e->h_ops.p + p.table_off);
@@ -773,6 +790,22 @@
     rc = resolve_child(e, b.key, b.leaf, prev_dst, &br->b, &br->b_sc, &st_unused, &br->b_kind);
     if (rc) return rc;
     br->len = len;
+    return IQHIP_OK;
+}
+
+int fill_image_submission(iqhip_engine *e) {
+    iqhip_engine::FillImage &f = e->fill_image;
+    f.use = false;
+    if (e->mfma || !f.on || !f.plan_hit || !e->plan.image_ok || e->plan.small) return IQHIP_OK;
+    if (f.model == e->model_version && f.buf.cap >= (size_t)e->plan.image_doubles) {
+        f.reused++;
+    } else {
+        if (f.buf.cap < (size_t)e->plan.image_doubles) HIPCHK(f.buf.ensure(e, (size_t)e->plan.image_doubles + 1024));
+        if (!e->planner) HIPCHK(launch_fill4_image(e, e->plan.small_nops));
+        f.model = e->model_version;
+        f.built++;
+    }
+    f.use = true;
     return IQHIP_OK;
 }
 
@@ -872,11 +905,14 @@
 int build_plan(iqhip_engine *e, const iqhip_node_op *ops, int nops, int *last_dst, const std::vector<int> *explicit_segs,
                const double *const *len_ptrs) {
     if (nops + 2 > e->result_cap) return fail(IQHIP_ERR_INVALID, "too many node updates in one submission");
+    e->fill_image.plan_hit = false;
     if (plan_is_cached(e, ops, nops, explicit_segs, len_ptrs)) {
         *last_dst = e->plan_cache.dst;
         mark_virtual_slabs(e);
+        e->fill_image.plan_hit = true;
         return IQHIP_OK;
     }
+    e->fill_image.model = 0;
     e->plan_cache.version = 0;
     if (e->staging_busy) {
         HIPCHK(hipEventSynchronize(e->staging_free));
diff --git a/iq-tree_amd/csrc/trav_phases.h b/iq-tree_amd/csrc/trav_phases.h
--- a/iq-tree_amd/csrc/trav_phases.h
+++ b/iq-tree_amd/csrc/trav_phases.h
@@ -59,4 +59,37 @@
 __device__ __forceinline__ double leaf_entry4(const double *Urow, const double *ex4, const double *tip4) {
     return leaf_e4(Urow, ex4).entry(tip4);
 }
+__device__ __forceinline__ double fill4_exp(const double *model, int e, double len) {
+    return exp(model[16 + (e & 3)] * (model[20 + (e >> 2)] * len));
 }
+__device__ __forceinline__ void fill4_leaf_table(double *reg, int B, int e, const double *model, const double *tip) {
+    const int c = e >> 2, x = e & 3;
+    const LeafE4 E = leaf_e4(model + x * 4, reg + c * 4);
+#pragma unroll
+    for (int row = 0; row < 4; row++) reg[B + row * B + e] = E.entry(tip + row * 4);
+    reg[B + 4 * B + e] = 1.0;
+}
+template <typename UPtr>
+__device__ __forceinline__ void fill4_pair_row(double *reg, int B, int c, int code, UPtr U, UPtr uinv) {
+    const int sa = code / 5, sb = code - 5 * sa;
+    const double *ta = reg + (2 + kPairRows + sa) * B + c * 4, *tb = reg + (8 + kPairRows + sb) * B + c * 4;
+    double tmp[4], l[4];
+#pragma unroll
+    for (int x = 0; x < 4; x++) tmp[x] = __dmul_rn(ta[x], tb[x]);
+#pragma unroll
+    for (int i = 0; i < 4; i++) {
+        double v = __dmul_rn(uinv[i * 4], tmp[0]);
+        v = fma(uinv[i * 4 + 1], tmp[1], v);
+        v = fma(uinv[i * 4 + 2], tmp[2], v);
+        v = fma(uinv[i * 4 + 3], tmp[3], v);
+        l[i] = __dmul_rn(reg[c * 4 + i], v);
+    }
+#pragma unroll
+    for (int x = 0; x < 4; x++) {
+        double v = __dmul_rn(U[x * 4], l[0]);
+        v = fma(U[x * 4 + 1], l[1], v);
+        v = fma(U[x * 4 + 2], l[2], v);
+        reg[B + code * B + c * 4 + x] = fma(U[x * 4 + 3], l[3], v);
+    }
+}
+}
```

Result: faster. 40000 M updates/s, median of 6 (+14.3%).
